# conservation-laws/ryujin

Hardware: AMD Instinct MI355X
Metric: MDoF-updates/s per Euler forward step; achieved HBM GB/s vs roofline (higher is better)
Workload: dtype f64; 1 GPU; 2D Euler Mach-3 forward-facing step, Q1, SSPRK33 stage sequence (BASELINE.json configs[1]); gridpoints_per_gpu=2498844, gridpoints_total=2498844, dofs_total=9995376, cells_per_unit=995, partition=x-slabs x1, equal gridpoint counts, develop_updates=600

## Files before the change

### include/ryujin_hip.h

```cpp
#ifndef RYUJIN_HIP_H
#define RYUJIN_HIP_H

#include <stddef.h>
#include <stdint.h>

#ifdef __cplusplus
extern "C" {
#endif

#define RYUJIN_OK 0
#define RYUJIN_WARN 1
#define RYUJIN_RESTART 2
#define RYUJIN_ERR_TAU (-1)
#define RYUJIN_ERR_ARG (-2)
#define RYUJIN_ERR_HIP (-3)
#define RYUJIN_ERR_COMM (-4)
#define RYUJIN_ERR_UNSUPPORTED (-5)

enum {
  RYUJIN_EQ_EULER = 0,
  RYUJIN_EQ_SHALLOW_WATER = 1,
  RYUJIN_EQ_EULER_AEOS = 2,
  RYUJIN_EQ_SCALAR_CONSERVATION = 3
};

enum { RYUJIN_FLUX_BURGERS = 0, RYUJIN_FLUX_KPP = 1, RYUJIN_FLUX_POLYNOMIAL = 2, RYUJIN_FLUX_FUNCTION = 3 };

enum {
  RYUJIN_EOS_POLYTROPIC_GAS = 0,
  RYUJIN_EOS_NOBLE_ABEL_STIFFENED_GAS = 1,
  RYUJIN_EOS_VAN_DER_WAALS = 2,
  RYUJIN_EOS_JONES_WILKINS_LEE = 3,
  RYUJIN_EOS_FUNCTION = 4
};

enum {
  RYUJIN_BC_DO_NOTHING = 0,
  RYUJIN_BC_PERIODIC = 1,
  RYUJIN_BC_SLIP = 2,
  RYUJIN_BC_NO_SLIP = 3,
  RYUJIN_BC_DIRICHLET = 4,
  RYUJIN_BC_DYNAMIC = 5,
  RYUJIN_BC_DIRICHLET_MOMENTUM = 6
};

enum { RYUJIN_IDV_WARN = 0, RYUJIN_IDV_RAISE_EXCEPTION = 1 };

typedef struct ryujin_hip_params {
  int equation;
  int dim;

  double gamma;
  double reference_density;
  double vacuum_state_relaxation_small;
  double vacuum_state_relaxation_large;

  double gravity;
  double manning_friction_coefficient;
  double reference_water_depth;
  double dry_state_relaxation_factor;
  double dry_state_relaxation_small;
  double dry_state_relaxation_large;

  double cfl;
  int id_violation_strategy;

  double indicator_evc_factor;

  int limiter_iterations;
  double limiter_newton_tolerance;
  int limiter_newton_max_iterations;
  double limiter_relaxation_factor;
  int limiter_limit_on_kinetic_energy;
  int limiter_limit_on_square_velocity;

  int riemann_newton_max_iterations;
  double riemann_newton_tolerance;

  int eos;
  int compute_strict_bounds;
  double eos_covolume_b;
  double eos_q;
  double eos_pinf;
  double eos_vdw_a;
  double eos_gas_constant_R;
  double jwl_A, jwl_B, jwl_R1, jwl_R2, jwl_omega, jwl_rho_0, jwl_q_0, jwl_cv;

  int sc_flux;
  double sc_flux_polynomial[3][4];
  double sc_derivative_approximation_delta;
  int sc_use_greedy_wavespeed;
  int sc_use_averaged_entropy;
  int sc_random_entropies;

  int system_scope_events;
  int debug_join_exchanges;
  int debug_bc_fold_max_slices;
  int debug_no_small_mesh_split;
  int debug_pij_storage;
  int debug_expensive_bounds_check;
  int debug_tile_map;
  int debug_band_stride;
  int debug_xcd_chunk;
  int debug_stencil_classes;
} ryujin_hip_params;

typedef struct ryujin_hip_offline {
  uint32_t n_export, n_internal, n_owned, n_relevant;
  uint32_t simd_length;
  const uint64_t *row_starts;
  const uint32_t *columns;
  const double *cij;
  const double *mij;
  const double *mi;
  const double *mi_inv;
  double measure_of_omega;

  uint32_t n_bdry;
  const uint32_t *b_i;
  const double *b_normal;
  const uint8_t *b_id;

  uint32_t n_pairs;
  const uint32_t *p_i, *p_col, *p_j;

  const double *initial_precomputed;

  int n_nbr;
  const int *nbr_rank;
  const uint32_t *send_off;
  const uint32_t *send_idx;
  const uint32_t *recv_off;
  const uint32_t *row_send_off;
  const uint32_t *row_send_row;
  const uint32_t *row_send_col;

  int discontinuous_ansatz;
  const double *incidence;
  const double *mass_matrix_inverse;
} ryujin_hip_offline;

typedef struct ryujin_hip_ctx ryujin_hip_ctx;

#define RYUJIN_HIP_UNIQUE_ID_BYTES 128
typedef struct ryujin_hip_comm ryujin_hip_comm;
int ryujin_hip_comm_unique_id(char id[RYUJIN_HIP_UNIQUE_ID_BYTES]);
int ryujin_hip_comm_init(ryujin_hip_comm **comm, const char id[RYUJIN_HIP_UNIQUE_ID_BYTES],
                         int rank, int n_ranks, int device);
int ryujin_hip_device_count(int *n_devices);
int ryujin_hip_comm_init_local(ryujin_hip_comm **comms, int n_ranks, int device);
int ryujin_hip_comm_init_loopback(ryujin_hip_comm **comm, int rank, int n_ranks, int device);
void ryujin_hip_comm_destroy(ryujin_hip_comm *comm);
int ryujin_hip_comm_info(const ryujin_hip_comm *comm, int *rank, int *n_ranks, int *rccl_rank,
                         int *rccl_count, int *rccl_device);

void ryujin_hip_default_params(ryujin_hip_params *params, int equation, int dim);

int ryujin_hip_create(ryujin_hip_ctx **ctx, const ryujin_hip_offline *offline,
                      const ryujin_hip_params *params, ryujin_hip_comm *comm, int device);
int ryujin_hip_exchange_info(ryujin_hip_ctx *ctx, int *n_nbr, int *nbr_rank, int max_nbr,
                             unsigned long long *n_exchanges, unsigned long long *n_allreduces);
void ryujin_hip_destroy(ryujin_hip_ctx *ctx);

int ryujin_hip_state_alloc(ryujin_hip_ctx *ctx, int *handle);
int ryujin_hip_state_free(ryujin_hip_ctx *ctx, int handle);
int ryujin_hip_state_upload(ryujin_hip_ctx *ctx, int handle, const double *U_aos);
int ryujin_hip_state_download(ryujin_hip_ctx *ctx, int handle, double *U_aos);
int ryujin_hip_state_download_precomputed(ryujin_hip_ctx *ctx, int handle, double *prec_aos);

int ryujin_hip_host_register(ryujin_hip_ctx *ctx, const void *ptr, size_t bytes);
int ryujin_hip_host_unregister(ryujin_hip_ctx *ctx, const void *ptr);
int ryujin_hip_state_download_owned(ryujin_hip_ctx *ctx, int handle, double *U_aos);
int ryujin_hip_state_download_prepared(ryujin_hip_ctx *ctx, int handle, double *U_aos);

int ryujin_hip_prepare_state_vector(ryujin_hip_ctx *ctx, int handle, double t,
                                    const double *dirichlet_aos);

int ryujin_hip_step(ryujin_hip_ctx *ctx, int h_old, int stages, const int *h_stage,
                    const double *stage_weights, int h_new, double tau_in,
                    double tau_max_in, double *tau_out);

int ryujin_hip_sadd(ryujin_hip_ctx *ctx, int h_dst, double s, double b, int h_src);

enum {
  RYUJIN_SCHEME_SSPRK_22 = 0,
  RYUJIN_SCHEME_SSPRK_33 = 1,
  RYUJIN_SCHEME_ERK_11 = 2,
  RYUJIN_SCHEME_ERK_22 = 3,
  RYUJIN_SCHEME_ERK_33 = 4,
  RYUJIN_SCHEME_ERK_43 = 5,
  RYUJIN_SCHEME_ERK_54 = 6
};
enum { RYUJIN_CFL_RECOVERY_NONE = 0, RYUJIN_CFL_RECOVERY_BANG_BANG = 1 };
int ryujin_hip_time_step(ryujin_hip_ctx *ctx, int scheme, int h_state, const int h_tmp[3],
                         const double *dirichlet_aos, double tau_max, int cfl_recovery, double cfl_min,
                         double cfl_max, double *tau_out);
int ryujin_hip_time_step_n(ryujin_hip_ctx *ctx, int scheme, int h_state, int n_tmp, const int *h_tmp,
                           const double *dirichlet_aos, double tau_max, int cfl_recovery,
                           double cfl_min, double cfl_max, double *tau_out);

typedef void (*ryujin_hip_dirichlet_fn)(void *user, double time, double *dirichlet_aos);
int ryujin_hip_time_step_fn(ryujin_hip_ctx *ctx, int scheme, int h_state, int n_tmp, const int *h_tmp, double t,
                            ryujin_hip_dirichlet_fn dirichlet_fn, void *user, double tau_max, int cfl_recovery,
                            double cfl_min, double cfl_max, double *tau_out);

int ryujin_hip_state_integrals(ryujin_hip_ctx *ctx, int handle, double *out );

int ryujin_hip_set_cfl(ryujin_hip_ctx *ctx, double cfl);
int ryujin_hip_get_cfl(ryujin_hip_ctx *ctx, double *cfl);
int ryujin_hip_set_id_violation_strategy(ryujin_hip_ctx *ctx, int strategy);
int ryujin_hip_get_alpha(ryujin_hip_ctx *ctx, double *alpha );
int ryujin_hip_get_counters(ryujin_hip_ctx *ctx, unsigned *n_restarts, unsigned *n_warnings);
int ryujin_hip_limiter_statistics(ryujin_hip_ctx *ctx, double *limited_slice_fraction, int *pij_stored,
                                  double *stored_slice_fraction);
int ryujin_hip_layout_info(ryujin_hip_ctx *ctx, unsigned long long *n_tiles, unsigned long long *n_regular_tiles);
int ryujin_hip_chain_info(ryujin_hip_ctx *ctx, unsigned long long *n_chained_tiles,
                          unsigned long long *n_chained_entries);
int ryujin_hip_stencil_class_info(ryujin_hip_ctx *ctx, unsigned long long *n_uniform_slices,
                                  unsigned long long *n_classes, double *uniform_entry_fraction);
int ryujin_hip_tile_statistics(ryujin_hip_ctx *ctx, double *stored_fraction, double *read_fraction,
                               double *formed_by_step6_fraction);

int ryujin_hip_debug_fetch(ryujin_hip_ctx *ctx, int what, double *out, size_t n_doubles);
#define RYUJIN_DEBUG_PLAN_LENGTH 32
int ryujin_hip_debug_plan(ryujin_hip_ctx *ctx, int *out, int n);
int ryujin_hip_set_timers(ryujin_hip_ctx *ctx, int enable);
int ryujin_hip_get_timers(ryujin_hip_ctx *ctx, double ms[8]);
int ryujin_hip_get_timers_accum(ryujin_hip_ctx *ctx, double ms[8], unsigned *n_updates, int reset);
int ryujin_hip_synchronize(ryujin_hip_ctx *ctx);
int ryujin_hip_event_record(ryujin_hip_ctx *ctx, int which );
int ryujin_hip_event_elapsed_ms(ryujin_hip_ctx *ctx, double *ms);
int ryujin_hip_debug_layout(const ryujin_hip_offline *offline, uint64_t *ptr, uint32_t *col,
                            uint64_t *transposed, const double *data, uint32_t n_comp, double *out);
int ryujin_hip_debug_addresses(ryujin_hip_ctx *ctx, uint64_t out[8]);
int ryujin_hip_debug_pow(int device, const double *x, const double *y, double *out, size_t n);
enum {
  RYUJIN_DEBUG_EULER_RIEMANN = 0,
  RYUJIN_DEBUG_EULER_LIMIT_1D = 1,
  RYUJIN_DEBUG_SW_RIEMANN = 2,
  RYUJIN_DEBUG_EULER_DIJ_2D = 3,
  RYUJIN_DEBUG_EULER_DIJ_3D = 4,
  RYUJIN_DEBUG_EULER_DIJ_RECORDS_2D = 5,
  RYUJIN_DEBUG_EULER_DIJ_RECORDS_3D = 6,
  RYUJIN_DEBUG_SW_DIJ_2D = 7,
  RYUJIN_DEBUG_SW_DIJ_RECORDS_2D = 8,
  RYUJIN_DEBUG_EULER_RIEMANN_RECORDS = 9,
  RYUJIN_DEBUG_SW_RIEMANN_RECORDS = 10,
  RYUJIN_DEBUG_AEOS_RIEMANN = 11,
  RYUJIN_DEBUG_AEOS_LIMIT_1D = 12,
  RYUJIN_DEBUG_AEOS_DIJ_2D = 13,
  RYUJIN_DEBUG_AEOS_DIJ_RECORDS_2D = 14,
  RYUJIN_DEBUG_EULER_LIMIT_CHECKED_1D = 15,
  RYUJIN_DEBUG_EULER_LIMIT_2D = 16
};
int ryujin_hip_debug_function(int device, const ryujin_hip_params *params, int which, const double *in,
                              double *out, size_t n);
int ryujin_hip_debug_rk_outcome(int restart_accum, int tau_invalid_accum, int id_violation_strategy);
const char *ryujin_hip_last_error(void);
const char *ryujin_hip_version(void);

#define RYUJIN_PP_MAX_QUANTITIES 8
enum { RYUJIN_PP_SCHLIEREN = 0, RYUJIN_PP_VORTICITY = 1 };
typedef struct ryujin_hip_postprocess_quantity {
  int kind;
  int is_primitive;
  int component;
} ryujin_hip_postprocess_quantity;
int ryujin_hip_postprocess_configure(ryujin_hip_ctx *ctx, int n_quantities,
                                     const ryujin_hip_postprocess_quantity *quantities, double beta,
                                     int recompute_bounds);
int ryujin_hip_postprocess_compute(ryujin_hip_ctx *ctx, int state_handle);
int ryujin_hip_postprocess_download(ryujin_hip_ctx *ctx, int q, double *out, int raw);
int ryujin_hip_postprocess_bounds(ryujin_hip_ctx *ctx, int q, double *q_max, double *q_min);

enum { RYUJIN_Q_INSTANTANEOUS = 1, RYUJIN_Q_TIME_AVERAGED = 2, RYUJIN_Q_SPACE_AVERAGED = 4 };
#define RYUJIN_Q_MAX_MANIFOLDS 16
#define RYUJIN_Q_NONE_YET 3
int ryujin_hip_quantities_add_manifold(ryujin_hip_ctx *ctx, uint32_t n_points, const uint32_t *index,
                                       const double *weight, int options, int *manifold_out);
int ryujin_hip_quantities_reset(ryujin_hip_ctx *ctx);
int ryujin_hip_quantities_clear_statistics(ryujin_hip_ctx *ctx);
int ryujin_hip_quantities_accumulate(ryujin_hip_ctx *ctx, int state_handle, double t);
int ryujin_hip_quantities_instantaneous(ryujin_hip_ctx *ctx, int manifold, int state_handle, double t, double *out);
int ryujin_hip_quantities_time_averaged(ryujin_hip_ctx *ctx, int manifold, double *out, double *t_begin,
                                        double *t_end);
int ryujin_hip_quantities_time_series(ryujin_hip_ctx *ctx, int manifold, double *rows, size_t capacity_rows,
                                      size_t *n_rows, int clear);

enum {
  RYUJIN_IV_UNIFORM = 0,
  RYUJIN_IV_RADIAL_CONTRAST = 1,
  RYUJIN_IV_ISENTROPIC_VORTEX = 2,
  RYUJIN_IV_LEBLANC = 3,
  RYUJIN_IV_RAREFACTION = 4,
  RYUJIN_IV_CIRCULAR_DAM_BREAK = 5,
  RYUJIN_IV_PARABOLOID = 6,
  RYUJIN_IV_RITTER_DAM_BREAK = 7,
  RYUJIN_IV_SMOOTH_VORTEX = 8,
  RYUJIN_IV_SLOPING_FRICTION = 9
};
typedef struct ryujin_hip_initial_values {
  int state;
  double params[16];
  double direction[3];
  double position[3];
  double perturbation;
// ... 58 lines not shown
```

### ryujin_amd/capi.py

```python
from __future__ import annotations

import ctypes as C
import os

import numpy as np

from . import _build

c_double_p = C.POINTER(C.c_double)
c_u32_p = C.POINTER(C.c_uint32)
c_u64_p = C.POINTER(C.c_uint64)
c_u8_p = C.POINTER(C.c_uint8)
c_int_p = C.POINTER(C.c_int)

RYUJIN_OK, RYUJIN_WARN, RYUJIN_RESTART = 0, 1, 2
RYUJIN_ERR_TAU, RYUJIN_ERR_ARG, RYUJIN_ERR_HIP, RYUJIN_ERR_COMM, RYUJIN_ERR_UNSUPPORTED = -1, -2, -3, -4, -5
EQ_EULER, EQ_SHALLOW_WATER, EQ_EULER_AEOS, EQ_SCALAR_CONSERVATION = 0, 1, 2, 3
FLUX_BURGERS, FLUX_KPP, FLUX_POLYNOMIAL, FLUX_FUNCTION = 0, 1, 2, 3
EOS_POLYTROPIC_GAS, EOS_NOBLE_ABEL_STIFFENED_GAS, EOS_VAN_DER_WAALS, EOS_JONES_WILKINS_LEE = 0, 1, 2, 3
EOS_FUNCTION = 4
EOS_PRESSURE, EOS_SPECIFIC_INTERNAL_ENERGY, EOS_TEMPERATURE, EOS_SPEED_OF_SOUND = 0, 1, 2, 3
BC_DO_NOTHING, BC_PERIODIC, BC_SLIP, BC_NO_SLIP, BC_DIRICHLET, BC_DYNAMIC, BC_DIRICHLET_MOMENTUM = range(7)
IDV_WARN, IDV_RAISE_EXCEPTION = 0, 1
CUT_NONE, CUT_BOX, CUT_CYLINDER = 0, 1, 2
SCHEME_SSPRK_22, SCHEME_SSPRK_33, SCHEME_ERK_11, SCHEME_ERK_22, SCHEME_ERK_33, SCHEME_ERK_43, SCHEME_ERK_54 = range(7)
CFL_RECOVERY_NONE, CFL_RECOVERY_BANG_BANG = 0, 1
UNIQUE_ID_BYTES = 128
DEBUG_EULER_RIEMANN, DEBUG_EULER_LIMIT_1D, DEBUG_SW_RIEMANN, DEBUG_EULER_DIJ_2D, DEBUG_EULER_DIJ_3D = range(5)
DEBUG_EULER_DIJ_RECORDS_2D, DEBUG_EULER_DIJ_RECORDS_3D = 5, 6
DEBUG_SW_DIJ_2D, DEBUG_SW_DIJ_RECORDS_2D = 7, 8
DEBUG_EULER_RIEMANN_RECORDS, DEBUG_SW_RIEMANN_RECORDS = 9, 10
DEBUG_AEOS_RIEMANN, DEBUG_AEOS_LIMIT_1D = 11, 12
DEBUG_AEOS_DIJ_2D, DEBUG_AEOS_DIJ_RECORDS_2D = 13, 14
DEBUG_EULER_LIMIT_CHECKED_1D, DEBUG_EULER_LIMIT_2D = 15, 16


DIRICHLET_FN = C.CFUNCTYPE(None, C.c_void_p, C.c_double, c_double_p)


class Params(C.Structure):
    _fields_ = [
        ("equation", C.c_int), ("dim", C.c_int),
        ("gamma", C.c_double), ("reference_density", C.c_double),
        ("vacuum_state_relaxation_small", C.c_double), ("vacuum_state_relaxation_large", C.c_double),
        ("gravity", C.c_double), ("manning_friction_coefficient", C.c_double),
        ("reference_water_depth", C.c_double), ("dry_state_relaxation_factor", C.c_double),
        ("dry_state_relaxation_small", C.c_double), ("dry_state_relaxation_large", C.c_double),
        ("cfl", C.c_double), ("id_violation_strategy", C.c_int),
        ("indicator_evc_factor", C.c_double),
        ("limiter_iterations", C.c_int), ("limiter_newton_tolerance", C.c_double),
        ("limiter_newton_max_iterations", C.c_int), ("limiter_relaxation_factor", C.c_double),
        ("limiter_limit_on_kinetic_energy", C.c_int), ("limiter_limit_on_square_velocity", C.c_int),
        ("riemann_newton_max_iterations", C.c_int), ("riemann_newton_tolerance", C.c_double),
        ("eos", C.c_int), ("compute_strict_bounds", C.c_int),
        ("eos_covolume_b", C.c_double), ("eos_q", C.c_double), ("eos_pinf", C.c_double),
        ("eos_vdw_a", C.c_double), ("eos_gas_constant_R", C.c_double),
        ("jwl_A", C.c_double), ("jwl_B", C.c_double), ("jwl_R1", C.c_double), ("jwl_R2", C.c_double),
        ("jwl_omega", C.c_double), ("jwl_rho_0", C.c_double), ("jwl_q_0", C.c_double),
        ("jwl_cv", C.c_double),
        ("sc_flux", C.c_int), ("sc_flux_polynomial", (C.c_double * 4) * 3),
        ("sc_derivative_approximation_delta", C.c_double), ("sc_use_greedy_wavespeed", C.c_int),
        ("sc_use_averaged_entropy", C.c_int), ("sc_random_entropies", C.c_int),
        ("system_scope_events", C.c_int), ("debug_join_exchanges", C.c_int),
        ("debug_bc_fold_max_slices", C.c_int), ("debug_no_small_mesh_split", C.c_int),
        ("debug_pij_storage", C.c_int), ("debug_expensive_bounds_check", C.c_int),
        ("debug_tile_map", C.c_int), ("debug_band_stride", C.c_int),
        ("debug_xcd_chunk", C.c_int), ("debug_stencil_classes", C.c_int),
    ]


class Offline(C.Structure):
    _fields_ = [
        ("n_export", C.c_uint32), ("n_internal", C.c_uint32), ("n_owned", C.c_uint32),
        ("n_relevant", C.c_uint32), ("simd_length", C.c_uint32),
        ("row_starts", c_u64_p), ("columns", c_u32_p), ("cij", c_double_p), ("mij", c_double_p),
        ("mi", c_double_p), ("mi_inv", c_double_p), ("measure_of_omega", C.c_double),
        ("n_bdry", C.c_uint32), ("b_i", c_u32_p), ("b_normal", c_double_p), ("b_id", c_u8_p),
        ("n_pairs", C.c_uint32), ("p_i", c_u32_p), ("p_col", c_u32_p), ("p_j", c_u32_p),
        ("initial_precomputed", c_double_p),
        ("n_nbr", C.c_int), ("nbr_rank", c_int_p), ("send_off", c_u32_p), ("send_idx", c_u32_p),
        ("recv_off", c_u32_p), ("row_send_off", c_u32_p), ("row_send_row", c_u32_p),
        ("row_send_col", c_u32_p),
        ("discontinuous_ansatz", C.c_int), ("incidence", c_double_p), ("mass_matrix_inverse", c_double_p),
    ]


class SynthSpec(C.Structure):
    _fields_ = [
        ("dim", C.c_int), ("n_cells", C.c_uint32 * 3), ("lower", C.c_double * 3),
        ("upper", C.c_double * 3), ("bc", C.c_int * 6), ("cut_kind", C.c_int),
        ("cut_lo", C.c_double * 3), ("cut_hi", C.c_double * 3), ("cyl_center", C.c_double * 2),
        ("cyl_radius", C.c_double), ("cut_bc", C.c_int), ("n_ranks", C.c_int), ("rank", C.c_int),
    ]


PP_SCHLIEREN, PP_VORTICITY = 0, 1
PP_MAX_QUANTITIES = 8
Q_INSTANTANEOUS, Q_TIME_AVERAGED, Q_SPACE_AVERAGED = 1, 2, 4
Q_MAX_MANIFOLDS = 16
Q_NONE_YET = 3
EN_MAX_DOFS_PER_CELL, EN_MAX_POINTS, EN_MAX_COMPONENTS = 27, 64, 5
OUT_MAX_QUANTITIES, OUT_MAX_MANIFOLDS = 32, 8
OUT_FLOAT32, OUT_FLOAT64 = 0, 1


class PostprocessQuantity(C.Structure):
    _fields_ = [("kind", C.c_int), ("is_primitive", C.c_int), ("component", C.c_int)]


(IV_UNIFORM, IV_RADIAL_CONTRAST, IV_ISENTROPIC_VORTEX, IV_LEBLANC, IV_RAREFACTION, IV_CIRCULAR_DAM_BREAK,
 IV_PARABOLOID, IV_RITTER_DAM_BREAK, IV_SMOOTH_VORTEX, IV_SLOPING_FRICTION) = range(10)


class InitialValues(C.Structure):
    _fields_ = [("state", C.c_int), ("params", C.c_double * 16), ("direction", C.c_double * 3),
                ("position", C.c_double * 3), ("perturbation", C.c_double)]


IV_STATES = {
    "uniform": (IV_UNIFORM, False, (("primitive state", 0, (1.4, 3.0, 1.0)),)),
    "radial contrast": (IV_RADIAL_CONTRAST, False, (("primitive state inner", 0, (1.0, 0.0, 100.0)),
                                                    ("primitive state outer", 3, (1.0, 0.0, 0.1)),
                                                    ("radius", 6, 0.5))),
    "isentropic vortex": (IV_ISENTROPIC_VORTEX, False, (("mach number", 0, 2.0), ("beta", 1, 5.0),
                                                        ("gamma", 2, 1.4))),
    "leblanc": (IV_LEBLANC, False, ()),
    "rarefaction": (IV_RAREFACTION, False, (("gamma", 0, 1.4),)),
    "circular dam break": (IV_CIRCULAR_DAM_BREAK, True, (("still water depth", 0, 0.5), ("radius", 1, 2.5),
                                                         ("dam amplitude", 2, 2.5))),
    "paraboloid": (IV_PARABOLOID, True, (("free surface radius", 0, 1.0), ("water height", 1, 0.1),
                                         ("paraboloid length", 2, 10000.0), ("speed", 3, 2.0))),
    "ritter dam break": (IV_RITTER_DAM_BREAK, True, (("time initial", 0, 0.1), ("left water depth", 1, 0.005))),
    "smooth vortex": (IV_SMOOTH_VORTEX, True, (("reference depth", 0, 1.0), ("mach number", 1, 2.0),
                                               ("beta", 2, 0.1))),
    "sloping friction": (IV_SLOPING_FRICTION, True, (("ramp slope", 0, 1.0), ("initial discharge", 1, 0.1))),
}


def initial_values_struct(name: str, dim: int, direction=None, position=None, perturbation: float = 0.0,
                          **params) -> InitialValues:
    if name not in IV_STATES:
        raise ValueError(f"Could not find an initial state description with name \"{name}\"")
    state, _, spec = IV_STATES[name]
    iv = InitialValues()
    iv.state = state
    given = {k.replace("_", " "): v for k, v in params.items()}
    for pname, slot, default in spec:
        value = given.pop(pname, default)
        values = tuple(value) if isinstance(default, tuple) else (value,)
        if len(values) != (len(default) if isinstance(default, tuple) else 1):
# ... 121 lines not shown

def resolve_component(equation: int, dim: int, name: str) -> tuple[int, int]:
    for is_primitive, names in enumerate(component_names(equation, dim)):
        if name in names:
            return is_primitive, names.index(name)
    raise ValueError(f"Invalid component name »{name}«")


def as_ptr(a: np.ndarray, typ):
    return a.ctypes.data_as(typ)


def np_from_ptr(ptr, n: int, dtype) -> np.ndarray:
    if n == 0 or not ptr:
        return np.zeros(0, dtype=dtype)
    return np.ctypeslib.as_array(ptr, shape=(n,)).astype(dtype, copy=True)



_synth = None


def load_synth():
    global _synth
    if _synth is None:
        path = os.environ.get("RYUJIN_SYNTH_LIB", _build.SYNTH_SO)
        if not os.path.exists(path):
            _build.build_synth()
        lib = C.CDLL(path)
        lib.ryujin_synth_build.restype = C.c_void_p
        lib.ryujin_synth_build.argtypes = [C.POINTER(SynthSpec)]
        lib.ryujin_synth_free.argtypes = [C.c_void_p]
        lib.ryujin_synth_last_error.restype = C.c_char_p
        lib.ryujin_synth_offline.restype = C.POINTER(Offline)
        lib.ryujin_synth_offline.argtypes = [C.c_void_p]
        lib.ryujin_synth_nnz.restype = C.c_uint64
        lib.ryujin_synth_nnz.argtypes = [C.c_void_p]
        lib.ryujin_synth_n_global.restype = C.c_uint64
        lib.ryujin_synth_n_global.argtypes = [C.c_void_p]
        lib.ryujin_synth_positions.restype = c_double_p
        lib.ryujin_synth_positions.argtypes = [C.c_void_p]
        lib.ryujin_synth_global_ids.restype = c_u64_p
        lib.ryujin_synth_global_ids.argtypes = [C.c_void_p]
        lib.ryujin_synth_bdry_positions.restype = c_double_p
        lib.ryujin_synth_bdry_positions.argtypes = [C.c_void_p]
        lib.ryujin_synth_bdry_mass.restype = c_double_p
        lib.ryujin_synth_bdry_mass.argtypes = [C.c_void_p]
        lib.ryujin_synth_n_cells.restype = C.c_uint64
        lib.ryujin_synth_n_cells.argtypes = [C.c_void_p]
        lib.ryujin_synth_cells.restype = c_u32_p
        lib.ryujin_synth_cells.argtypes = [C.c_void_p]
        lib.ryujin_synth_ghost_row_send_entries.restype = C.c_size_t
        lib.ryujin_synth_ghost_row_send_entries.argtypes = [c_u64_p, c_u32_p, c_u32_p, C.c_size_t, C.c_uint32,
                                                            C.c_uint32, c_u32_p, c_u32_p]
        lib.ryujin_offline_write.restype = C.c_int
        lib.ryujin_offline_write.argtypes = [C.c_char_p, C.POINTER(Offline), C.c_int, C.c_int, c_double_p,
                                             c_double_p]
        lib.ryujin_offline_read.restype = C.c_void_p
        lib.ryujin_offline_read.argtypes = [C.c_char_p]
        lib.ryujin_offline_file_free.argtypes = [C.c_void_p]
        lib.ryujin_offline_io_last_error.restype = C.c_char_p
        lib.ryujin_offline_file_view.restype = C.POINTER(Offline)
        lib.ryujin_offline_file_view.argtypes = [C.c_void_p]
        lib.ryujin_offline_file_dim.argtypes = [C.c_void_p]
        lib.ryujin_offline_file_n_initial_precomputed.argtypes = [C.c_void_p]
        lib.ryujin_offline_file_nnz.restype = C.c_uint64
        lib.ryujin_offline_file_nnz.argtypes = [C.c_void_p]
        lib.ryujin_offline_file_positions.restype = c_double_p
        lib.ryujin_offline_file_positions.argtypes = [C.c_void_p]
        lib.ryujin_offline_file_b_positions.restype = c_double_p
        lib.ryujin_offline_file_b_positions.argtypes = [C.c_void_p]
        _synth = lib
    return _synth



HIP_SYMBOLS = [
    "ryujin_hip_comm_unique_id", "ryujin_hip_comm_init", "ryujin_hip_comm_init_local",
    "ryujin_hip_comm_init_loopback",
    "ryujin_hip_comm_destroy", "ryujin_hip_comm_info", "ryujin_hip_exchange_info", "ryujin_hip_device_count",
    "ryujin_hip_time_step_fn", "ryujin_hip_debug_addresses",
    "ryujin_hip_host_register", "ryujin_hip_host_unregister", "ryujin_hip_state_download_owned",
    "ryujin_hip_state_download_prepared", "ryujin_hip_layout_info", "ryujin_hip_chain_info", "ryujin_hip_stencil_class_info", "ryujin_hip_tile_statistics",
    "ryujin_hip_default_params", "ryujin_hip_create", "ryujin_hip_destroy",
    "ryujin_hip_state_alloc", "ryujin_hip_state_free", "ryujin_hip_state_upload",
    "ryujin_hip_state_download", "ryujin_hip_state_download_precomputed", "ryujin_hip_state_integrals",
    "ryujin_hip_prepare_state_vector", "ryujin_hip_step", "ryujin_hip_sadd", "ryujin_hip_time_step", "ryujin_hip_time_step_n",
    "ryujin_hip_get_timers_accum",
    "ryujin_hip_set_cfl", "ryujin_hip_get_cfl", "ryujin_hip_set_id_violation_strategy",
    "ryujin_hip_get_alpha", "ryujin_hip_get_counters", "ryujin_hip_limiter_statistics", "ryujin_hip_debug_fetch", "ryujin_hip_debug_plan",
    "ryujin_hip_set_timers", "ryujin_hip_get_timers", "ryujin_hip_synchronize",
    "ryujin_hip_event_record", "ryujin_hip_event_elapsed_ms", "ryujin_hip_last_error",
    "ryujin_hip_version", "ryujin_hip_debug_layout", "ryujin_hip_debug_pow", "ryujin_hip_debug_function", "ryujin_hip_debug_rk_outcome",
    "ryujin_hip_postprocess_configure", "ryujin_hip_postprocess_compute", "ryujin_hip_postprocess_download",
    "ryujin_hip_postprocess_bounds",
    "ryujin_hip_quantities_add_manifold", "ryujin_hip_quantities_reset", "ryujin_hip_quantities_clear_statistics",
    "ryujin_hip_quantities_accumulate", "ryujin_hip_quantities_instantaneous", "ryujin_hip_quantities_time_averaged",
    "ryujin_hip_quantities_time_series",
    "ryujin_hip_initial_values_configure", "ryujin_hip_initial_values_evaluate",
    "ryujin_hip_initial_values_interpolate", "ryujin_hip_prepare_state_vector_iv", "ryujin_hip_time_step_iv",
    "ryujin_hip_initial_values_configure_function", "ryujin_hip_expression_evaluate",
    "ryujin_hip_error_norms_configure", "ryujin_hip_error_norms_compute",
    "ryujin_hip_flux_configure_function", "ryujin_hip_flux_function_evaluate", "ryujin_hip_flux_info",
    "ryujin_hip_eos_configure_function", "ryujin_hip_eos_function_evaluate",
    "ryujin_hip_eos_function_evaluate_device", "ryujin_hip_eos_info",
    "ryujin_hip_output_configure", "ryujin_hip_output_info", "ryujin_hip_output_selection",
    "ryujin_hip_output_levelset_values", "ryujin_hip_output_extract",
]


def _declare_module_api(lib, prefix: str):
    p = lambda n: getattr(lib, prefix + n)
    vp = C.c_void_p
    p("default_params").argtypes = [C.POINTER(Params), C.c_int, C.c_int]
    p("default_params").restype = None
    p("create").argtypes = [C.POINTER(vp), C.POINTER(Offline), C.POINTER(Params), vp, C.c_int]
    p("destroy").argtypes = [vp]
    p("destroy").restype = None
    p("state_alloc").argtypes = [vp, c_int_p]
    p("state_free").argtypes = [vp, C.c_int]
    p("state_upload").argtypes = [vp, C.c_int, c_double_p]
    p("state_download").argtypes = [vp, C.c_int, c_double_p]
    p("state_download_precomputed").argtypes = [vp, C.c_int, c_double_p]
    if hasattr(lib, prefix + "state_integrals"):
        p("state_integrals").argtypes = [vp, C.c_int, c_double_p]
    p("prepare_state_vector").argtypes = [vp, C.c_int, C.c_double, c_double_p]
    p("step").argtypes = [vp, C.c_int, C.c_int, c_int_p, c_double_p, C.c_int, C.c_double,
                          C.c_double, c_double_p]
    p("sadd").argtypes = [vp, C.c_int, C.c_double, C.c_double, C.c_int]
    p("set_cfl").argtypes = [vp, C.c_double]
    p("get_cfl").argtypes = [vp, c_double_p]
    p("set_id_violation_strategy").argtypes = [vp, C.c_int]
    p("get_alpha").argtypes = [vp, c_double_p]
    p("get_counters").argtypes = [vp, C.POINTER(C.c_uint), C.POINTER(C.c_uint)]
    p("debug_fetch").argtypes = [vp, C.c_int, c_double_p, C.c_size_t]
    p("last_error").restype = C.c_char_p


_hip = None


def load_hip():
    global _hip
    if _hip is None:
        path = os.environ.get("RYUJIN_HIP_LIB", _build.HIP_SO)
        if not os.path.exists(path):
            raise RuntimeError(
                f"{path} is missing: build it with `python -m ryujin_amd._build` "
                "(hipcc --offload-arch=gfx950). There is no CPU fallback for the product path.")
        lib = C.CDLL(path, mode=C.RTLD_GLOBAL)
        _declare_module_api(lib, "ryujin_hip_")
        vp = C.c_void_p
        lib.ryujin_hip_comm_unique_id.argtypes = [C.c_char_p]
        lib.ryujin_hip_comm_init.argtypes = [C.POINTER(vp), C.c_char_p, C.c_int, C.c_int, C.c_int]
        lib.ryujin_hip_comm_init_local.argtypes = [C.POINTER(vp), C.c_int, C.c_int]
        lib.ryujin_hip_comm_init_loopback.argtypes = [C.POINTER(vp), C.c_int, C.c_int, C.c_int]
        lib.ryujin_hip_comm_destroy.argtypes = [vp]
        lib.ryujin_hip_comm_destroy.restype = None
        lib.ryujin_hip_comm_info.argtypes = [vp, c_int_p, c_int_p, c_int_p, c_int_p, c_int_p]
        lib.ryujin_hip_exchange_info.argtypes = [vp, c_int_p, c_int_p, C.c_int, C.POINTER(C.c_ulonglong),
                                                 C.POINTER(C.c_ulonglong)]
        lib.ryujin_hip_set_timers.argtypes = [vp, C.c_int]
        lib.ryujin_hip_get_timers.argtypes = [vp, c_double_p]
        lib.ryujin_hip_get_timers_accum.argtypes = [vp, c_double_p, C.POINTER(C.c_uint), C.c_int]
        lib.ryujin_hip_time_step.argtypes = [vp, C.c_int, C.c_int, c_int_p, c_double_p, C.c_double, C.c_int,
                                             C.c_double, C.c_double, c_double_p]
        lib.ryujin_hip_time_step_n.argtypes = [vp, C.c_int, C.c_int, C.c_int, c_int_p, c_double_p, C.c_double,
                                               C.c_int, C.c_double, C.c_double, c_double_p]
        lib.ryujin_hip_time_step_fn.argtypes = [vp, C.c_int, C.c_int, C.c_int, c_int_p, C.c_double, DIRICHLET_FN,
                                                C.c_void_p, C.c_double, C.c_int, C.c_double, C.c_double, c_double_p]
        lib.ryujin_hip_device_count.argtypes = [c_int_p]
        lib.ryujin_hip_layout_info.argtypes = [vp, C.POINTER(C.c_ulonglong), C.POINTER(C.c_ulonglong)]
        lib.ryujin_hip_chain_info.argtypes = [vp, C.POINTER(C.c_ulonglong), C.POINTER(C.c_ulonglong)]
        if hasattr(lib, "ryujin_hip_stencil_class_info"):
            lib.ryujin_hip_stencil_class_info.argtypes = [vp, C.POINTER(C.c_ulonglong), C.POINTER(C.c_ulonglong),
                                                          C.POINTER(C.c_double)]
        lib.ryujin_hip_tile_statistics.argtypes = [vp, C.POINTER(C.c_double), C.POINTER(C.c_double), C.POINTER(C.c_double)]
        lib.ryujin_hip_host_register.argtypes = [vp, C.c_void_p, C.c_size_t]
        lib.ryujin_hip_host_unregister.argtypes = [vp, C.c_void_p]
        lib.ryujin_hip_state_download_owned.argtypes = [vp, C.c_int, c_double_p]
        lib.ryujin_hip_state_download_prepared.argtypes = [vp, C.c_int, c_double_p]
        lib.ryujin_hip_debug_addresses.argtypes = [vp, c_u64_p]
        lib.ryujin_hip_debug_plan.argtypes = [vp, c_int_p, C.c_int]
        lib.ryujin_hip_synchronize.argtypes = [vp]
        lib.ryujin_hip_event_record.argtypes = [vp, C.c_int]
        lib.ryujin_hip_event_elapsed_ms.argtypes = [vp, c_double_p]
        lib.ryujin_hip_version.restype = C.c_char_p
        lib.ryujin_hip_debug_layout.argtypes = [C.POINTER(Offline), c_u64_p, c_u32_p, c_u64_p,
                                                c_double_p, C.c_uint32, c_double_p]
        lib.ryujin_hip_debug_pow.argtypes = [C.c_int, c_double_p, c_double_p, c_double_p, C.c_size_t]
        lib.ryujin_hip_debug_rk_outcome.argtypes = [C.c_int, C.c_int, C.c_int]
        lib.ryujin_hip_debug_function.argtypes = [C.c_int, C.POINTER(Params), C.c_int, c_double_p, c_double_p,
                                                  C.c_size_t]
        lib.ryujin_hip_postprocess_configure.argtypes = [vp, C.c_int, C.POINTER(PostprocessQuantity), C.c_double,
                                                         C.c_int]
        lib.ryujin_hip_postprocess_compute.argtypes = [vp, C.c_int]
        lib.ryujin_hip_postprocess_download.argtypes = [vp, C.c_int, c_double_p, C.c_int]
        lib.ryujin_hip_postprocess_bounds.argtypes = [vp, C.c_int, c_double_p, c_double_p]
        lib.ryujin_hip_quantities_add_manifold.argtypes = [vp, C.c_uint32, c_u32_p, c_double_p, C.c_int, c_int_p]
        lib.ryujin_hip_quantities_reset.argtypes = [vp]
        lib.ryujin_hip_quantities_clear_statistics.argtypes = [vp]
        lib.ryujin_hip_quantities_accumulate.argtypes = [vp, C.c_int, C.c_double]
        lib.ryujin_hip_quantities_instantaneous.argtypes = [vp, C.c_int, C.c_int, C.c_double, c_double_p]
        lib.ryujin_hip_quantities_time_averaged.argtypes = [vp, C.c_int, c_double_p, c_double_p, c_double_p]
        lib.ryujin_hip_quantities_time_series.argtypes = [vp, C.c_int, c_double_p, C.c_size_t,
                                                          C.POINTER(C.c_size_t), C.c_int]
        lib.ryujin_hip_initial_values_configure.argtypes = [vp, C.POINTER(InitialValues), c_double_p, c_double_p]
        lib.ryujin_hip_initial_values_evaluate.argtypes = [vp, c_double_p, C.c_size_t, C.c_double, c_double_p]
        lib.ryujin_hip_initial_values_interpolate.argtypes = [vp, C.c_int, C.c_double]
        lib.ryujin_hip_prepare_state_vector_iv.argtypes = [vp, C.c_int, C.c_double]
        lib.ryujin_hip_time_step_iv.argtypes = [vp, C.c_int, C.c_int, C.c_int, c_int_p, C.c_double, C.c_double,
                                                C.c_int, C.c_double, C.c_double, c_double_p]
        lib.ryujin_hip_initial_values_configure_function.argtypes = [vp, C.c_int, C.POINTER(C.c_char_p), c_double_p,
                                                                     c_double_p, c_double_p, c_double_p]
        lib.ryujin_hip_expression_evaluate.argtypes = [C.c_char_p, C.c_int, c_double_p, C.c_size_t, C.c_double,
                                                       c_double_p]
        lib.ryujin_hip_error_norms_configure.argtypes = [vp, C.c_uint32, C.c_int, c_u32_p, C.c_int, c_double_p,
                                                         c_double_p, c_double_p, C.c_int]
        lib.ryujin_hip_error_norms_compute.argtypes = [vp, C.c_int, C.c_int, C.c_int, c_int_p, C.c_int, c_double_p,
                                                       c_double_p]
        lib.ryujin_hip_flux_configure_function.argtypes = [vp, C.c_char_p, C.c_double]
        lib.ryujin_hip_flux_function_evaluate.argtypes = [C.c_char_p, C.c_int, C.c_double, c_double_p, C.c_size_t,
                                                          c_double_p, c_double_p]
        lib.ryujin_hip_flux_info.argtypes = [vp, c_int_p, c_int_p, c_int_p]
        lib.ryujin_hip_eos_configure_function.argtypes = [vp, C.c_char_p, C.c_char_p, C.c_char_p, C.c_char_p,
                                                          C.c_double, C.c_double, C.c_double]
        lib.ryujin_hip_eos_function_evaluate.argtypes = [C.c_int, C.c_char_p, c_double_p, c_double_p, C.c_size_t,
                                                         c_double_p]
        lib.ryujin_hip_eos_function_evaluate_device.argtypes = [vp, C.c_int, c_double_p, c_double_p, C.c_size_t,
                                                                c_double_p]
        lib.ryujin_hip_eos_info.argtypes = [vp, c_int_p, c_int_p, c_int_p]
        lib.ryujin_hip_output_configure.argtypes = [vp, C.c_int, C.POINTER(C.c_char_p), c_double_p, C.c_uint32, C.c_int,
                                                    c_u32_p, C.c_int, C.POINTER(C.c_char_p)]
        lib.ryujin_hip_output_info.argtypes = [vp, c_u32_p, c_u32_p]
        lib.ryujin_hip_output_selection.argtypes = [vp, c_u32_p, c_u32_p, c_u32_p]
        lib.ryujin_hip_output_levelset_values.argtypes = [vp, C.c_int, c_double_p]
        lib.ryujin_hip_output_extract.argtypes = [vp, C.c_int, C.c_int, C.c_int, C.c_void_p]
        _hip = lib
    return _hip
```

### ryujin_amd/csrc/kernels_euler.hpp

```cpp

#pragma once

#include <hip/hip_runtime.h>

#include <cfloat>
#include <cstdint>

#include "euler_device.hpp"

namespace ryujin_hip
{
  struct DeviceScalars;

  struct StencilClassEntry {
    double c[2];
    double m;
    int32_t delta;
    uint32_t pad;
  };
  static_assert(sizeof(StencilClassEntry) == 32, "four 64-bit words");

  struct StepBegin {
    DeviceScalars *scalars;
    double tau_max_in, tau_in;
// ... 311 lines not shown
    const v4i v = *(const_ptr)(uintptr_t)(M.class_table + e);
    c[0] = uniform_double(v.x, v.y);
    if constexpr (DIM == 2)
      c[1] = uniform_double(v.z, v.w);
  }

  RYUJIN_DEV int32_t class_delta(const DeviceMesh &M, const uint32_t e)
  {
    typedef const int32_t __attribute__((address_space(4))) *const_ptr;
    return __builtin_amdgcn_readfirstlane(*(const_ptr)(uintptr_t)(&M.class_table[e].delta));
  }

  struct TileChain {
    uint32_t kind;
    uint64_t loads;
  };
  template <int DIM>
  constexpr bool chain_masks_pay()
  {
    return DIM == 3;
  }
  template <bool MASKS>
  RYUJIN_DEV TileChain tile_chain(const DeviceMesh &M, const uint64_t colbase)
  {
    TileChain t{kChainNone, ~0ull};
    if (M.tiles != nullptr) {
      typedef const uint32_t __attribute__((address_space(4))) *const_ptr;
      typedef const uint64_t __attribute__((address_space(4))) *const_ptr64;
      const uint32_t code = __builtin_amdgcn_readfirstlane(*(const_ptr)(uintptr_t)&M.tiles[colbase].chain);
      if constexpr (MASKS) {
        t.kind = code & kChainKindMask;
        if (t.kind != kChainNone) {
          const uint64_t m = *(const_ptr64)(uintptr_t)(M.chain_loads + colbase);
          t.loads = ((uint64_t)__builtin_amdgcn_readfirstlane((uint32_t)(m >> 32)) << 32) |
                    (uint64_t)__builtin_amdgcn_readfirstlane((uint32_t)m);
        }
      } else {
        t.kind = (code & kChainEndLaneOnly) != 0u ? (code & kChainKindMask) : kChainNone;
      }
    }
    return t;
  }

  RYUJIN_DEV double lane_next(const double x)
  {
    const int lo = __double2loint(x), hi = __double2hiint(x);
    return __hiloint2double(__builtin_amdgcn_update_dpp(hi, hi, 0x130 , 0xf, 0xf, false),
                            __builtin_amdgcn_update_dpp(lo, lo, 0x130, 0xf, 0xf, false));
  }
  RYUJIN_DEV double lane_prev(const double x)
  {
    const int lo = __double2loint(x), hi = __double2hiint(x);
    return __hiloint2double(__builtin_amdgcn_update_dpp(hi, hi, 0x138 , 0xf, 0xf, false),
                            __builtin_amdgcn_update_dpp(lo, lo, 0x138, 0xf, 0xf, false));
  }
  template <bool MASKS>
  RYUJIN_DEV bool chain_lane_loads(const TileChain &t, const uint32_t lane)
  {
    if constexpr (MASKS)
      return ((t.loads >> lane) & 1ull) != 0ull;
    else
      return lane == (t.kind == kChainOwnPrev ? 0u : 63u);
  }

  RYUJIN_DEV uint32_t tile_transposed(const DeviceMesh &M, const TileDesc &t, const uint64_t colbase,
                                      const uint32_t lane)
  {
    if (t.delta != kTileIrregular)
      return (lane < 64u - ((uint32_t)t.delta & 63u) ? t.ta : t.tb) + lane;
    uint32_t pos = M.idx_t[colbase * 64 + lane];
    asm volatile("" : "+v"(pos));
    return pos;
  }

  template <bool USE = true>
  RYUJIN_DEV uint32_t tile_transposed(const DeviceMesh &M, const uint64_t colbase, const uint32_t lane)
  {
    return tile_transposed(M, tile_desc<USE>(M, colbase), colbase, lane);
  }

  RYUJIN_DEV void batch_fence() { __builtin_amdgcn_sched_barrier(0); }

  template <bool USE, int N>
  RYUJIN_DEV void transposed_positions(const DeviceMesh &M, const RowCtx &r, const int c0, uint32_t (&tpos)[N])
  {
    if constexpr (USE) {
      if (M.tiles != nullptr) {
        int4 raw[N];
#pragma unroll
        for (int k = 0; k < N; ++k) {
          raw[k] = int4{kTileIrregular, 0, 0, 0};
          if ((uint32_t)(c0 + k) < r.width)
            raw[k] = load_tile_desc(M.tiles + ((uint64_t)r.base + c0 + k));
        }
        batch_fence();
        bool any_irregular = false;
#pragma unroll
        for (int k = 0; k < N; ++k) {
          tpos[k] = 0;
          if ((uint32_t)(c0 + k) < r.width) {
            const int32_t delta = __builtin_amdgcn_readfirstlane(raw[k].x);
            const uint32_t ta = (uint32_t)__builtin_amdgcn_readfirstlane(raw[k].y);
            const uint32_t tb = (uint32_t)__builtin_amdgcn_readfirstlane(raw[k].z);
            tpos[k] = (r.lane < 64u - ((uint32_t)delta & 63u) ? ta : tb) + r.lane;
            any_irregular = any_irregular || delta == kTileIrregular;
          }
        }
        if (any_irregular) {
#pragma unroll
          for (int k = 0; k < N; ++k)
            if ((uint32_t)(c0 + k) < r.width && __builtin_amdgcn_readfirstlane(raw[k].x) == kTileIrregular)
              tpos[k] = M.idx_t[((uint64_t)r.base + c0 + k) * 64 + r.lane];
        }
#pragma unroll
        for (int k = 0; k < N; ++k)
          asm volatile("" : "+v"(tpos[k]));
        return;
      }
    }
#pragma unroll
    for (int k = 0; k < N; ++k) {
      tpos[k] = 0;
      if ((uint32_t)(c0 + k) < r.width)
        tpos[k] = M.idx_t[((uint64_t)r.base + c0 + k) * 64 + r.lane];
    }
#pragma unroll
    for (int k = 0; k < N; ++k)
      asm volatile("" : "+v"(tpos[k]));
  }

  RYUJIN_DEV void arrived(double &x) { asm volatile("" : "+v"(x)); }
  RYUJIN_DEV void arrived(uint32_t &x) { asm volatile("" : "+v"(x)); }
  template <int N>
  RYUJIN_DEV void arrived(double (&x)[N])
  {
#pragma unroll
    for (int q = 0; q < N; ++q)
      arrived(x[q]);
  }

  RYUJIN_DEV uint32_t mapped_block(const DeviceMesh &M)
  {
    uint32_t block = blockIdx.x;
    if (M.xcd_chunk > 0u) {
      const uint32_t span = 8u * M.xcd_chunk;
      if (block < gridDim.x - gridDim.x % span) {
        const uint32_t rem = block % span;
        block = block - rem + (rem & 7u) * M.xcd_chunk + (rem >> 3);
      }
    }
    return block;
  }

  RYUJIN_DEV RowCtx row_context(const DeviceMesh &M)
  {
    RowCtx r;
    r.lane = threadIdx.x & 63;
    const uint32_t block = mapped_block(M);
    uint32_t id = block * kWavesPerBlock + (uint32_t)__builtin_amdgcn_readfirstlane(threadIdx.x >> 6);
    if (M.band_stride > 1u) {
      const uint32_t band = kWavesPerBlock * M.band_stride;
      const uint32_t n = M.slice_end - M.slice_begin;
      if (id < n - n % band) {
        const uint32_t rem = id % band;
        id = id - rem + rem / kWavesPerBlock + (rem % kWavesPerBlock) * M.band_stride;
      }
    }
    r.slice = __builtin_amdgcn_readfirstlane(M.slice_begin + id);
    r.valid = r.slice < M.slice_end;
    if (!r.valid) {
      r.row = r.len = r.base = r.width = 0;
      return r;
    }
    r.row = r.slice * 64 + r.lane;
    r.len = M.row_len[r.row];
    r.base = __builtin_amdgcn_readfirstlane(M.slice_off[r.slice]);
    r.width = __builtin_amdgcn_readfirstlane(M.slice_off[r.slice + 1]) - r.base;
    return r;
  }


  struct BcFold {
    const unsigned long long *slice_mask;
    const uint32_t *slice_first;
    const uint32_t *grp_start;
    const double *b_normal;
    const uint8_t *b_id;
    const double *dirichlet;
  };

  template <typename E>
  RYUJIN_DEV void apply_bc_group(const typename E::Params &P, const BcFold &B, const uint32_t g, const uint32_t i,
                                 double *U)
  {
    constexpr int K = E::K;
    constexpr int DIM = E::DIMENSION;
    const uint32_t e0 = B.grp_start[g], e1 = B.grp_start[g + 1];
    double U_i[K];
    load_state<K>(U, i, U_i);
    bool touched = false;
    for (uint32_t e = e0; e < e1; ++e) {
      const int id = B.b_id[e];
      if (id == RYUJIN_BC_DO_NOTHING)
        continue;
      double normal[DIM], U_D[K], result[K];
#pragma unroll
// ... 934 lines not shown
```

### ryujin_amd/csrc/kernels_limiter.hpp

```cpp

#pragma once

#include "kernels_euler.hpp"


namespace ryujin_hip
{
  RYUJIN_DEV double lmin(const double a, const double b)
  {
    return (a == a && b == b) ? fmin(a, b) : a + b;
  }

  RYUJIN_DEV void flag_restart(DeviceScalars *scalars, const bool all_ok, const uint32_t lane)
  {
    if (__any(!all_ok)) {
      if (lane == 0)
        atomicOr(&scalars->restart_needed, 1);
    }
  }

  template <typename E>
  struct TailScratch {
    static constexpr int kRowDoubles = (E::NB + E::K) * 64;
    double rows[kRowDoubles];
// ... 636 lines not shown
          if (!__any(active && !(old_l_ij == 1.))) {
            if (active)
              st_stream(lij_next + (pos), 0.);
            continue;
          }
          double p_ij[K];
          load_entry<K>(pij, colbase, r.lane, p_ij);
          if (!active)
            continue;
          double new_p_ij[K];
#pragma unroll
          for (int q = 0; q < K; ++q)
            new_p_ij[q] = (1. - old_l_ij) * p_ij[q];
          bool success, undecided;
          const double new_l_ij =
              E::limit_fast(P, bnd, U_i_new, new_p_ij, success, undecided);
          if (undecided)
            undecided_mask |= 1ull << (c - c_blk + 1);
          else
            st_stream(lij_next + (pos), (1. - old_l_ij) * new_l_ij);
        }
        limit_undecided_pairs<E>(
            P, r, undecided_mask, bnd, U_i_new, tail_queue + (threadIdx.x >> 6) * 63 * 64,
            tail_rows[threadIdx.x >> 6].rows,
            [&](const uint32_t c, const uint32_t owner, double (&out)[K]) {
              const uint64_t pos = ((uint64_t)r.base + c) * 64 + owner;
              const double old_l_ij = lmin(lij[pos], lij[idx_t[pos]]);
              load_entry<K>(pij, (uint64_t)r.base + c, owner, out);
#pragma unroll
              for (int q = 0; q < K; ++q)
                out[q] = (1. - old_l_ij) * out[q];
            },
            [&](const uint32_t c, const uint32_t owner, const double new_l_ij) {
              const uint64_t pos = ((uint64_t)r.base + c) * 64 + owner;
              const double old_l_ij = lmin(lij[pos], lij[idx_t[pos]]);
              st_stream(lij_next + (pos), (1. - old_l_ij) * new_l_ij);
            },
            c_blk - 1);
        undecided_mask = 0;
        if constexpr (!WIDE)
          break;
      }
    }
  }

  template <int K>
  RYUJIN_DEV void repair_missing_tiles(const uint32_t *__restrict__ cols, const double *__restrict__ mij,
                                       const double *__restrict__ mi_inv, const double *__restrict__ old_U,
                                       const double *__restrict__ r_in, const double *__restrict__ alpha,
                                       const double *__restrict__ dij, const double tau, const uint32_t i,
                                       const uint32_t len, const uint32_t base, const uint32_t width,
                                       const uint32_t lane, const bool row_active, const uint32_t missing,
                                       double *__restrict__ pij)
  {
    RowData<K> row;
    load_state<K>(old_U, i, row.U_i);
    load_state<K>(r_in, i, row.F_i);
    row.alpha_i = alpha[i];
    row.m_i_inv = mi_inv[i];
    row.factor = tau * row.m_i_inv * (double)(len - 1);
#pragma unroll 1
    for (uint32_t c = 1; c < width; ++c) {
      if (!((missing >> c) & 1u))
        continue;
      const uint64_t pos = ((uint64_t)base + c) * 64 + lane;
      const uint32_t j = cols[pos];
      PairData<K> pd;
      pd.d_ij = dij[pos];
      pd.m_ij = ld_stream(mij + pos);
      load_state<K>(old_U, j, pd.U_j);
      load_state<K>(r_in, j, pd.F_j);
      pd.alpha_j = alpha[j];
      pd.m_j_inv = mi_inv[j];
      double P_t[K];
      pij_stage0<K>(row, pd, P_t);
      if (row_active && c < len)
        store_entry<K>(pij, (uint64_t)base + c, lane, P_t);
    }
  }

  struct SliceFlags {
    uint8_t *unlimited, *first_stored, *todo;
    uint32_t *needed_tiles;
  };

#ifndef RYUJIN_GATHER_GROUP_3D
#define RYUJIN_GATHER_GROUP_3D 6
#endif
  template <int MAXW>
  RYUJIN_DEV uint32_t tiles_predicted(const SliceFlags &W, const uint32_t slice)
  {
    static_assert(MAXW <= 10, "P_ij per tile up to two dimensions");
    const uint32_t word = W.needed_tiles[slice];
    uint32_t m = word & 0x3ffu;
    m |= (word >> 10) & 0x3ffu;
    m |= (word >> 20) & 0x3ffu;
    return m;
  }
  template <int MAXW>
  RYUJIN_DEV void tiles_remember(const SliceFlags &W, const uint32_t slice, const uint32_t needed)
  {
    static_assert(MAXW <= 10, "P_ij per tile up to two dimensions");
    W.needed_tiles[slice] = ((W.needed_tiles[slice] << 10) | (needed & 0x3ffu)) & 0x3fffffffu;
  }

  template <int K>
  RYUJIN_DEV void backfill_pij(const DeviceMesh &M, const Stage0Src &S0, const RowCtx &r,
                               double *__restrict__ pij, const uint32_t c_end)
  {
    if (r.len <= 1)
      return;
    RowData<K> row;
    load_row_data<K>(M, S0, r.row, r.len, row);
    for (uint32_t c = 1; c < c_end && c < r.len; ++c) {
      double P_ij[K];
      pij_on_the_fly<K>(M, S0, row, (uint64_t)r.base + c, r.lane, P_ij);
      store_entry<K>(pij, (uint64_t)r.base + c, r.lane, P_ij);
    }
  }

  template <typename E, int MAXW, int CHUNK>
  RYUJIN_DEV void last_cached_slice(const typename E::Params &P, const DeviceMesh &M, const RowCtx &r,
                                    double *__restrict__ new_U, const double *__restrict__ pij,
                                    const double *__restrict__ lij, const FusedSadd &F, const FusedPrecompute &FP,
                                    const uint8_t *__restrict__ slice_unlimited = nullptr)
  {
    constexpr int K = E::K;
    const bool row_active = r.len > 1;
    const uint32_t i = row_active ? r.row : (r.row < M.n_owned ? r.row : M.n_owned - 1);
    const uint32_t *__restrict__ idx_t = M.idx_t;

    double U_i_new[K];
    load_state<K>(new_U, i, U_i_new);
    double V[K];
    if (F.src)
      load_state<K>(F.src, i, V);
    const double lambda = 1. / (double)(r.len - 1);

    double l[MAXW];
    uint32_t needed = 0;
    const bool known_unlimited = slice_unlimited != nullptr && slice_unlimited[r.slice] != 0;
#pragma unroll
    for (int c = 1; c < MAXW; ++c)
      l[c] = 0.;
    if (!known_unlimited) {
      constexpr int CH = MAXW - 1 < 9 ? MAXW - 1 : RYUJIN_GATHER_GROUP_3D;
#pragma unroll
      for (int c0 = 1; c0 < MAXW; c0 += CH) {
        uint32_t tpos[CH];
        transposed_positions<tile_map_pays<E::DIMENSION>(), CH>(M, r, c0, tpos);
        batch_fence();
        double l_a[CH], l_b[CH];
#pragma unroll
        for (int k = 0; k < CH; ++k) {
          const int c = c0 + k;
          l_a[k] = l_b[k] = 0.;
          if (c < MAXW && (uint32_t)c < r.width) {
            l_a[k] = lij[(uint32_t)(((uint64_t)r.base + c) * 64 + r.lane)];
            l_b[k] = lij[tpos[k]];
          }
        }
        batch_fence();
#pragma unroll
        for (int k = 0; k < CH; ++k) {
          asm volatile("" : "+v"(l_a[k]));
          asm volatile("" : "+v"(l_b[k]));
        }
#pragma unroll
        for (int k = 0; k < CH; ++k) {
          const int c = c0 + k;
          if (c < MAXW && (uint32_t)c < r.width)
            l[c] = (row_active && (uint32_t)c < r.len) ? lmin(l_a[k], l_b[k]) : 0.;
        }
      }
#pragma unroll
      for (int c = 1; c < MAXW; ++c)
        if (__any(l[c] != 0.))
          needed |= 1u << c;
    }

#pragma unroll
    for (int c0 = 1; c0 < MAXW; c0 += CHUNK) {
      double p[CHUNK][K];
#pragma unroll
      for (int cc = 0; cc < CHUNK; ++cc) {
        const int c = c0 + cc;
        if (c < MAXW && ((needed >> c) & 1u))
          load_entry<K>(pij, (uint64_t)r.base + c, r.lane, p[cc]);
      }
#pragma unroll
      for (int cc = 0; cc < CHUNK; ++cc) {
        const int c = c0 + cc;
        if (c < MAXW && ((needed >> c) & 1u)) {
          if (row_active && (uint32_t)c < r.len) {
#pragma unroll
            for (int q = 0; q < K; ++q)
              U_i_new[q] += l[c] * lambda * p[cc][q];
          }
        }
      }
    }

    if (F.src) {
#pragma unroll
      for (int q = 0; q < K; ++q)
        U_i_new[q] = F.s * U_i_new[q] + F.b * V[q];
    }
    if (row_active || (F.src != nullptr && r.row < M.n_owned))
      store_state<K>(new_U, i, U_i_new);
    if (FP.prec != nullptr && row_active)
      fused_precompute<E>(P, FP, i, U_i_new);
  }

  RYUJIN_DEV RowCtx row_context_of_slice(const DeviceMesh &M, const uint32_t slice)
  {
    RowCtx r;
    r.lane = threadIdx.x & 63;
    r.slice = slice;
    r.valid = true;
    r.row = slice * 64 + r.lane;
    r.len = M.row_len[r.row];
    r.base = M.slice_off[slice];
    r.width = M.slice_off[slice + 1] - r.base;
    return r;
  }

  template <typename E, int MAXW, int CHUNK>
  __global__ void __launch_bounds__(kBlock, (MAXW > 9 ? RYUJIN_OCC_LAST_3D : 1))
  k_high_order_last_cached(const typename E::Params P, const DeviceMesh M, double *__restrict__ new_U,
                           const double *__restrict__ pij, const double *__restrict__ lij, const FusedSadd F,
                           const FusedPrecompute FP, const uint8_t *__restrict__ slice_unlimited = nullptr)
  {
    const RowCtx r = row_context(M);
    if (!r.valid)
      return;
    last_cached_slice<E, MAXW, CHUNK>(P, M, r, new_U, pij, lij, F, FP, slice_unlimited);
  }

  constexpr int kHoPlain = 0, kHoLight = 1, kHoHeavy = 2;
  template <int DIM, int MODE>
  constexpr bool forms_missing_tiles()
  {
    return DIM <= 2 && MODE == kHoPlain;
  }

  template <typename E, int MAXW, int CP, bool SPLIT, int MODE>
  RYUJIN_DEV void next_cached_slice(const typename E::Params &P, const DeviceMesh &M, const RowCtx &r,
                                    const uint32_t group, double *__restrict__ new_U,
                                    const double *__restrict__ bounds, double *__restrict__ pij,
                                    const double *__restrict__ lij, double *__restrict__ lij_next,
                                    const double *__restrict__ V_unlimited, const Stage0Src &S0, const SliceFlags &W,
                                    const uint32_t todo = 1)
  {
    constexpr int K = E::K;
    constexpr int NB = E::NB;
    static_assert(!SPLIT || CP == MAXW, "the split variant caches the whole row");
    static_assert(!SPLIT || MODE == kHoPlain, "small meshes keep the stored P_ij");
    const bool row_active = r.len > 1;
    const uint32_t i = row_active ? r.row : (r.row < M.n_owned ? r.row : M.n_owned - 1);
    const uint32_t *__restrict__ idx_t = M.idx_t;

    double l[MAXW];
    if constexpr (MODE == kHoLight) {
      bool limited = false;
      constexpr int CH = MAXW - 1 < 9 ? MAXW - 1 : RYUJIN_GATHER_GROUP_3D;
#pragma unroll
      for (int c0 = 1; c0 < MAXW; c0 += CH) {
        uint32_t tpos[CH];
        transposed_positions<tile_map_pays<E::DIMENSION>(), CH>(M, r, c0, tpos);
        batch_fence();
        double l_a[CH], l_b[CH];
#pragma unroll
        for (int k = 0; k < CH; ++k) {
          const int c = c0 + k;
          l_a[k] = l_b[k] = 1.;
          if (c < MAXW && (uint32_t)c < r.width) {
            l_a[k] = lij[(uint32_t)(((uint64_t)r.base + c) * 64 + r.lane)];
            l_b[k] = lij[tpos[k]];
          }
        }
        batch_fence();
#pragma unroll
        for (int k = 0; k < CH; ++k) {
          asm volatile("" : "+v"(l_a[k]));
          asm volatile("" : "+v"(l_b[k]));
        }
#pragma unroll
        for (int k = 0; k < CH; ++k) {
          const int c = c0 + k;
          if (c < MAXW && (uint32_t)c < r.width)
            limited = limited || (row_active && (uint32_t)c < r.len && !(l_a[k] == 1. && l_b[k] == 1.));
        }
      }
      const bool slice_limited = __any(limited);
      if ((r.slice & 15u) == 0 && r.lane == 0) {
        atomicAdd(&S0.scalars->n_sampled_slices, 1u);
        if (slice_limited)
          atomicAdd(&S0.scalars->n_sampled_limited, 1u);
      }
      if (r.lane == 0) {
        W.todo[r.slice] = slice_limited ? 3 : 0;
        if (!slice_limited)
          W.unlimited[r.slice] = 1;
      }
      if (!slice_limited && row_active) {
        double V_i[K];
        load_state<K>(V_unlimited, i, V_i);
        store_state<K>(new_U, i, V_i);
#pragma unroll
        for (int c = 1; c < MAXW; ++c)
          if ((uint32_t)c < r.len)
            st_stream(lij_next + ((r.base + c) * 64 + r.lane), 0.);
      }
      return;
    }

    double U_i_new[K];
    const double lambda = 1. / (double)(r.len - 1);
    const size_t stride = M.bounds_stride;
    double bnd[NB];
#pragma unroll
    for (int b = 0; b < NB; ++b)
      bnd[b] = bounds[(size_t)b * stride + i];

    double p[CP][K];
    uint32_t needed = 0;
    uint32_t own_limited = 0;
    if (V_unlimited != nullptr) {
      constexpr bool kTileMode = forms_missing_tiles<E::DIMENSION, MODE>() && !SPLIT;
      const bool tiles = kTileMode && S0.tile_store != 0 && W.needed_tiles != nullptr;
      uint32_t predicted = 0u;
      if constexpr (kTileMode)
        predicted = tiles ? tiles_predicted<MAXW>(W, r.slice) : 0u;
      bool limited = false;
      auto fetch_l = [&](const uint32_t lane) {
        needed = own_limited = 0u;
        constexpr int CH = MAXW - 1 < 9 ? MAXW - 1 : RYUJIN_GATHER_GROUP_3D;
        RowCtx rr = r;
        rr.lane = lane;
#pragma unroll
        for (int c0 = 1; c0 < MAXW; c0 += CH) {
          uint32_t tpos[CH];
          transposed_positions<tile_map_pays<E::DIMENSION>(), CH>(M, rr, c0, tpos);
          batch_fence();
          double l_a[CH], l_b[CH];
#pragma unroll
          for (int k = 0; k < CH; ++k) {
            const int c = c0 + k;
            l_a[k] = l_b[k] = 1.;
            if (c < MAXW && (uint32_t)c < r.width) {
              l_a[k] = lij[(uint32_t)(((uint64_t)r.base + c) * 64 + lane)];
              l_b[k] = lij[tpos[k]];
            }
          }
          batch_fence();
#pragma unroll
          for (int k = 0; k < CH; ++k) {
            asm volatile("" : "+v"(l_a[k]));
            asm volatile("" : "+v"(l_b[k]));
          }
#pragma unroll
          for (int k = 0; k < CH; ++k) {
            const int c = c0 + k;
            if (c >= MAXW)
              continue;
            l[c] = 1.;
            if ((uint32_t)c < r.width) {
              const bool lane_on = row_active && (uint32_t)c < r.len;
              const bool lim = lane_on && !(l_a[k] == 1. && l_b[k] == 1.);
              l[c] = lane_on ? lmin(l_a[k], l_b[k]) : 1.;
              limited = limited || lim;
              if (__any(lim))
                needed |= 1u << c;
              if (__any(lane_on && !(l_a[k] == 1.)))
                own_limited |= 1u << c;
            }
          }
        }
      };
      fetch_l(r.lane);
      const bool slice_limited = needed != 0u;
      (void)limited;
      const uint32_t missing = (kTileMode && S0.tile_store != 0) ? (needed & ~(own_limited | predicted)) : 0u;
      if (S0.scalars != nullptr && (r.slice & 15u) == 0 && r.lane == 0 && (!SPLIT || group == 0) &&
          !(MODE == kHoHeavy && todo == 3)) {
        atomicAdd(&S0.scalars->n_sampled_slices, 1u);
        if (slice_limited)
          atomicAdd(&S0.scalars->n_sampled_limited, 1u);
      }
      if (W.unlimited != nullptr && r.lane == 0 && (!SPLIT || group == 0))
        W.unlimited[r.slice] = slice_limited ? 0 : 1;
      if constexpr (kTileMode)
        if (tiles && r.lane == 0 && (!SPLIT || group == 0))
          tiles_remember<MAXW>(W, r.slice, needed);
      load_state<K>(V_unlimited, i, U_i_new);
      if (!slice_limited) {
        if (row_active) {
          if (!SPLIT || group == 0)
            store_state<K>(new_U, i, U_i_new);
#pragma unroll
          for (int c = 1; c < MAXW; ++c)
            if ((uint32_t)c < r.len && (!SPLIT || (uint32_t)(c - 1) % kWavesPerBlock == group))
              st_stream(lij_next + ((r.base + c) * 64 + r.lane), 0.);
        }
        return;
      }
      if (kTileMode && tiles && (r.slice & 15u) == 0 && r.lane == 0 && (!SPLIT || group == 0)) {
        atomicAdd(&S0.scalars->n_sampled_tiles_needed, (unsigned int)__popc(needed));
        atomicAdd(&S0.scalars->n_sampled_tiles_formed, (unsigned int)__popc(missing));
      }
      if constexpr (kTileMode) {
        if (missing != 0u)
          repair_missing_tiles<K>(M.cols, M.mij, M.mi_inv, S0.old_U, S0.r_in, S0.alpha, S0.dij, S0.scalars->tau, i,
                                  r.len, r.base, r.width, r.lane, row_active, missing, pij);
      }
      if constexpr (E::kLimitedUpdateFromV) {
        const uint32_t row_cols = row_active ? ((r.len >= 32u ? 0xffffffffu : ((1u << r.len) - 1u)) & ~1u) : 0u;
        const bool ref_order = row_active && (needed & row_cols) == row_cols;
        if (__any(ref_order)) {
          double U_low[K];
          load_state<K>(new_U, i, U_low);
#pragma unroll
          for (int q = 0; q < K; ++q)
            U_i_new[q] = ref_order ? U_low[q] : U_i_new[q];
        }
#pragma unroll
        for (int c = 1; c < CP; ++c) {
#pragma unroll
          for (int q = 0; q < K; ++q)
            p[c][q] = 0.;
          if ((needed >> c) & 1u)
            load_entry<K>(pij, (uint64_t)r.base + c, r.lane, p[c]);
        }
#pragma unroll
        for (int c = 1; c < MAXW; ++c) {
          if (!((needed >> c) & 1u))
            continue;
          const double w = (row_active && (uint32_t)c < r.len) ? (ref_order ? l[c] : l[c] - 1.) : 0.;
          if (c < CP) {
#pragma unroll
            for (int q = 0; q < K; ++q)
              U_i_new[q] += w * lambda * p[c < CP ? c : 0][q];
          } else {
            double pt[K];
            load_entry<K>(pij, (uint64_t)r.base + c, r.lane, pt);
#pragma unroll
            for (int q = 0; q < K; ++q)
              U_i_new[q] += w * lambda * pt[q];
          }
        }
      } else {
        load_state<K>(new_U, i, U_i_new);
#pragma unroll
        for (int c = 1; c < CP; ++c) {
#pragma unroll
          for (int q = 0; q < K; ++q)
            p[c][q] = 0.;
          if ((uint32_t)c < r.width)
            load_entry<K>(pij, (uint64_t)r.base + c, r.lane, p[c]);
        }
#pragma unroll
        for (int c = 1; c < MAXW; ++c) {
          if (c < CP) {
            if (row_active && (uint32_t)c < r.len) {
#pragma unroll
              for (int q = 0; q < K; ++q)
                U_i_new[q] += l[c] * lambda * p[c < CP ? c : 0][q];
            }
          } else if ((uint32_t)c < r.width) {
            double pt[K];
            load_entry<K>(pij, (uint64_t)r.base + c, r.lane, pt);
            if (row_active && (uint32_t)c < r.len) {
#pragma unroll
              for (int q = 0; q < K; ++q)
                U_i_new[q] += l[c] * lambda * pt[q];
            }
          }
        }
      }
    } else {
      load_state<K>(new_U, i, U_i_new);
#pragma unroll
      for (int c = 1; c < MAXW; ++c) {
        l[c] = 0.;
        if (c < CP) {
#pragma unroll
          for (int q = 0; q < K; ++q)
            p[c < CP ? c : 0][q] = 0.;
        }
        if ((uint32_t)c < r.width) {
          const uint64_t colbase = (uint64_t)r.base + c;
          const uint32_t pos = (uint32_t)(colbase * 64 + r.lane);
          const double l_a = lij[pos];
          const double l_b = lij[tile_transposed<tile_map_pays<E::DIMENSION>()>(M, (uint64_t)r.base + c, r.lane)];
          l[c] = lmin(l_a, l_b);
          if (c < CP)
            load_entry<K>(pij, colbase, r.lane, p[c < CP ? c : 0]);
          if (__any(row_active && (uint32_t)c < r.len && !(l[c] == 1.)))
            needed |= 1u << c;
        }
      }
#pragma unroll
      for (int c = 1; c < MAXW; ++c) {
        if (c < CP) {
          if (row_active && (uint32_t)c < r.len) {
#pragma unroll
            for (int q = 0; q < K; ++q)
              U_i_new[q] += l[c] * lambda * p[c < CP ? c : 0][q];
          }
        } else if ((uint32_t)c < r.width) {
          double pt[K];
          load_entry<K>(pij, (uint64_t)r.base + c, r.lane, pt);
          if (row_active && (uint32_t)c < r.len) {
#pragma unroll
            for (int q = 0; q < K; ++q)
              U_i_new[q] += l[c] * lambda * pt[q];
          }
        }
      }
    }
    if constexpr (SPLIT) {
      __syncthreads();
      if (row_active && group == 0)
        store_state<K>(new_U, i, U_i_new);
    } else {
      if (row_active)
        store_state<K>(new_U, i, U_i_new);
    }

    unsigned long long undecided_mask = 0;
#pragma unroll
    for (int c = 1; c < MAXW; ++c) {
      if ((uint32_t)c >= r.width)
        continue;
      if (SPLIT && (uint32_t)(c - 1) % kWavesPerBlock != group)
        continue;
      const bool lane_on = row_active && (uint32_t)c < r.len;
      if (!((needed >> c) & 1u)) {
        if (lane_on)
          st_stream(lij_next + ((r.base + c) * 64 + r.lane), 0.);
        continue;
      }
      double pc[K];
      if (c < CP) {
#pragma unroll
        for (int q = 0; q < K; ++q)
          pc[q] = p[c < CP ? c : 0][q];
      } else {
        load_entry<K>(pij, (uint64_t)r.base + c, r.lane, pc);
      }
      if (lane_on) {
        double new_p_ij[K];
#pragma unroll
        for (int q = 0; q < K; ++q)
          new_p_ij[q] = (1. - l[c]) * pc[q];
        bool success, undecided;
        const double new_l_ij =
            E::limit_fast(P, bnd, U_i_new, new_p_ij, success, undecided);
        if (undecided)
          undecided_mask |= 1ull << c;
        else
          st_stream(lij_next + ((r.base + c) * 64 + r.lane), (1. - l[c]) * new_l_ij);
      }
    }
    __shared__ uint16_t tail_queue[kWavesPerBlock * (MAXW - 1) * 64];
    __shared__ TailScratch<E> tail_rows[kWavesPerBlock];
    limit_undecided_pairs<E>(
        P, r, undecided_mask, bnd, U_i_new, tail_queue + (threadIdx.x >> 6) * (MAXW - 1) * 64,
        tail_rows[threadIdx.x >> 6].rows,
        [&](const uint32_t c, const uint32_t owner, double (&out)[K]) {
          const uint64_t pos = ((uint64_t)r.base + c) * 64 + owner;
          const double old_l_ij = lmin(lij[pos], lij[idx_t[pos]]);
          load_entry<K>(pij, (uint64_t)r.base + c, owner, out);
#pragma unroll
          for (int q = 0; q < K; ++q)
            out[q] = (1. - old_l_ij) * out[q];
        },
        [&](const uint32_t c, const uint32_t owner, const double new_l_ij) {
          const uint64_t pos = ((uint64_t)r.base + c) * 64 + owner;
          const double old_l_ij = lmin(lij[pos], lij[idx_t[pos]]);
          st_stream(lij_next + (pos), (1. - old_l_ij) * new_l_ij);
        });
  }

  template <typename E>
  __global__ void __launch_bounds__(kBlock)
  k_pij_repair(const DeviceMesh M, const Stage0Src S0, double *__restrict__ pij, const SliceFlags W)
  {
    const uint32_t slice = M.slice_begin + blockIdx.x * kWavesPerBlock + (threadIdx.x >> 6);
    if (slice >= M.slice_end || W.todo[slice] < 2)
      return;
    const uint32_t fs = W.first_stored[slice];
    const RowCtx r = row_context_of_slice(M, slice);
    backfill_pij<E::K>(M, S0, r, pij, fs == 0 ? 0xffffffffu : fs);
    if (r.lane == 0)
      W.first_stored[slice] = 1;
  }

  template <typename E, int MAXW, int CP = MAXW, bool SPLIT = false, int MODE = kHoPlain>
  __global__ void __launch_bounds__(kBlock, (MAXW > 9 ? (CP < MAXW ? RYUJIN_OCC_HO_3D : 1) : RYUJIN_OCC_HO))
  k_high_order_next_cached(const typename E::Params P, const DeviceMesh M, double *__restrict__ new_U,
                           const double *__restrict__ bounds, double *__restrict__ pij,
                           const double *__restrict__ lij, double *__restrict__ lij_next,
                           const double *__restrict__ V_unlimited = nullptr, const Stage0Src S0 = Stage0Src{},
                           const SliceFlags W = SliceFlags{})
  {
    RowCtx r;
    const uint32_t group = SPLIT ? (threadIdx.x >> 6) : 0u;
    uint32_t todo = 1;
    if constexpr (SPLIT) {
      if (M.slice_begin + blockIdx.x >= M.slice_end)
        return;
      r = row_context_of_slice(M, M.slice_begin + blockIdx.x);
    } else if constexpr (MODE == kHoLight || MODE == kHoHeavy) {
      const uint32_t slice = M.slice_begin + mapped_block(M) * kWavesPerBlock + (threadIdx.x >> 6);
      if (slice >= M.slice_end)
        return;
      if constexpr (MODE == kHoLight) {
        const uint32_t fs = W.first_stored[slice];
        if (fs != 0) {
          if ((threadIdx.x & 63) == 0)
            W.todo[slice] = fs == 1 ? 1 : 2;
          return;
        }
      } else {
        todo = W.todo[slice];
        if (todo == 0)
          return;
      }
      r = row_context_of_slice(M, slice);
    } else {
      r = row_context(M);
      if (!r.valid)
        return;
    }
    next_cached_slice<E, MAXW, CP, SPLIT, MODE>(P, M, r, group, new_U, bounds, pij, lij, lij_next, V_unlimited, S0,
                                                W, todo);
  }
}
```

### ryujin_amd/csrc/ryujin_hip.hip

```cpp

#include <hip/hip_runtime.h>
#include <rccl/rccl.h>

#include <algorithm>
#include <atomic>
#include <cmath>
#include <cstddef>
#include <cstdlib>
#include <cstring>
#include <condition_variable>
#include <limits>
#include <memory>
#include <mutex>
#include <numeric>
#include <string>
#include <type_traits>
#include <vector>

#include "ryujin_hip.h"

#ifndef RYUJIN_XCD_CHUNK_3D
#define RYUJIN_XCD_CHUNK_3D 8
#endif

// ... 371 lines not shown
    DeviceBuffer<uint32_t> d_cell_dofs;
    DeviceBuffer<double> d_jxw;
    DeviceBuffer<double> d_shape, d_weights;
    DeviceBuffer<double> d_work;
  };
  std::unique_ptr<ErrorNorms> error_norms;
  void error_norms_compute(int h_state, int h_analytic, const ErrorNormsDesc &D, double *host_result);
  struct Output {
    OutputDesc desc{};
    bool needs_precomputed = false, needs_postprocessed = false;
    int n_postprocess = 0, pp_kind[kPostprocessMaxQuantities] = {}, pp_select[kPostprocessMaxQuantities] = {};
    int n_manifolds = 0, dofs_per_cell = 0;
    uint32_t n_cells = 0, n_selected_cells = 0, n_selected_nodes = 0;
    DeviceBuffer<double> d_levelsets;
    DeviceBuffer<uint32_t> d_cell_ids, d_node_ids, d_connectivity;
    DeviceBuffer<double> d_columns;
    DeviceBuffer<OutputDesc> d_desc;
    DeviceBuffer<unsigned char> d_out;
  };
  std::unique_ptr<Output> output;
  template <typename E>
  void output_extract(Output &o, int h, bool levelsets, bool float64, void *host_out);
  static constexpr int kMaxRkStages = 5;
  unsigned long long *h_tau_early = nullptr;
  hipEvent_t ev_tau = nullptr;
  bool want_tau_early = false;
  double *h_dirichlet_stage[kMaxRkStages] = {};
  bool iv_configured = false;
  InitialValuesParams iv{};
  DeviceBuffer<double> d_iv_positions, d_iv_b_positions;
  DeviceBuffer<IvFunctionProgram> d_iv_function;
  DeviceBuffer<double> d_iv_points, d_iv_values;
  struct IvStage {
    bool on;
    double t, c;
  };
  void require_initial_values() const
  {
    if (!iv_configured)
      throw HipError(RYUJIN_ERR_ARG, "initial values: not configured (ryujin_hip_initial_values_configure)");
  }
  template <typename E>
  void initial_values_points(const double *d_points, size_t n, double t, int stride, double *d_out);

  struct State {
    DeviceBuffer<double> U, prec;
    DeviceBuffer<double> rrec;
    bool used = false;
    bool precomputed = false;
    bool prepared = false;
  };
  std::vector<std::unique_ptr<State>> states;

  ExchangeTables exch;
  DeviceBuffer<uint32_t> d_send_idx, d_row_send_pos;
  DeviceBuffer<double> d_send_buf;

  DeviceBuffer<double> d_V;
  StepPlan last_plan{};
  Stage0Src last_s0{};
  struct LaunchRecord {
    uint32_t n_slices = 0, grid_y = 0;
    bool shares_slices = false;
  };
  struct LaunchLog {
    static constexpr int kParts = 2;
    int n_step5 = 0, n_step6 = 0;
    LaunchRecord step5[kParts], step6[kParts];
  } last_launches{};
  void record_step5(const DeviceMesh &mm, const uint32_t grid_y)
  {
    if (last_launches.n_step5 < LaunchLog::kParts)
      last_launches.step5[last_launches.n_step5] = LaunchRecord{mm.slice_end - mm.slice_begin, grid_y, false};
    ++last_launches.n_step5;
  }
  void record_step6(const DeviceMesh &mm, const uint32_t grid_y, const bool shares_slices)
  {
    if (last_launches.n_step6 < LaunchLog::kParts)
      last_launches.step6[last_launches.n_step6] = LaunchRecord{mm.slice_end - mm.slice_begin, grid_y, shares_slices};
    ++last_launches.n_step6;
  }
  DeviceBuffer<uint8_t> d_slice_unlimited, d_slice_first_stored, d_slice_todo;
  DeviceBuffer<uint32_t> d_slice_needed;
  double limited_fraction = 1., stored_fraction = 1.;
  unsigned int seen_sampled_slices = 0, seen_sampled_limited = 0, seen_sampled_stored = 0;
  unsigned int seen_sampled_tiles = 0, seen_sampled_tiles_stored = 0;
  unsigned int seen_sampled_tiles_needed = 0, seen_sampled_tiles_formed = 0;
  double tiles_needed_fraction = 1., tiles_formed_fraction = 0.;
  void update_limited_fraction()
  {
    const unsigned int d_tiles = h_scalars->n_sampled_tiles - seen_sampled_tiles;
    const unsigned int d_tiles_stored = h_scalars->n_sampled_tiles_stored - seen_sampled_tiles_stored;
    seen_sampled_tiles = h_scalars->n_sampled_tiles;
    seen_sampled_tiles_stored = h_scalars->n_sampled_tiles_stored;
    const unsigned int d_slices = h_scalars->n_sampled_slices - seen_sampled_slices;
    const unsigned int d_limited = h_scalars->n_sampled_limited - seen_sampled_limited;
    const unsigned int d_stored = h_scalars->n_sampled_stored - seen_sampled_stored;
    seen_sampled_slices = h_scalars->n_sampled_slices;
    seen_sampled_limited = h_scalars->n_sampled_limited;
    seen_sampled_stored = h_scalars->n_sampled_stored;
    if (d_slices != 0) {
      limited_fraction = (double)d_limited / (double)d_slices;
      stored_fraction = last_plan.per_slice() ? (double)d_stored / (double)d_slices : 1.;
    }
    const unsigned int d_needed = h_scalars->n_sampled_tiles_needed - seen_sampled_tiles_needed;
    const unsigned int d_formed = h_scalars->n_sampled_tiles_formed - seen_sampled_tiles_formed;
    seen_sampled_tiles_needed = h_scalars->n_sampled_tiles_needed;
    seen_sampled_tiles_formed = h_scalars->n_sampled_tiles_formed;
    if (last_plan.per_tile() && d_tiles != 0) {
      stored_fraction = (double)d_tiles_stored / (double)d_tiles;
      tiles_needed_fraction = (double)d_needed / (double)d_tiles;
      tiles_formed_fraction = (double)d_formed / (double)d_tiles;
    }
  }
  void ensure_pij()
  {
    if (d_pij.n == 0)
      d_pij.alloc(L.nnz_total * (size_t)K);
  }
  template <typename E>
  void store_pij_for_debug();

  unsigned n_restarts = 0, n_warnings = 0;
  unsigned long long n_exchanges = 0, n_allreduces = 0;

  bool timers_enabled = false;
  bool deferred = false;
  int rk_stage = 0;
  double sweep_ms_accum[8] = {};
  unsigned sweep_updates_accum = 0;
  hipEvent_t ev_rk[5][9] = {};
  hipEvent_t ev[9] = {};
  hipEvent_t ev_user[2] = {};
  double sweep_ms[8] = {};

  ~ryujin_hip_ctx()
  {
    if (stream)
      (void)hipStreamSynchronize(stream);
    if (comm_stream) {
      (void)hipStreamSynchronize(comm_stream);
      (void)hipStreamDestroy(comm_stream);
    }
    if (ev_prev)
      (void)hipEventDestroy(ev_prev);
    if (ev_exp)
      (void)hipEventDestroy(ev_exp);
    if (ev_comm)
      (void)hipEventDestroy(ev_comm);
    for (auto &e : ev)
      if (e)
        (void)hipEventDestroy(e);
    for (auto &set : ev_rk)
      for (auto &e : set)
        if (e)
          (void)hipEventDestroy(e);
    for (auto &e : ev_user)
      if (e)
        (void)hipEventDestroy(e);
    if (h_scalars)
      (void)hipHostFree(h_scalars);
    if (h_bc_pack)
      (void)hipHostFree(h_bc_pack);
    for (const void *ptr : registered_host)
      (void)hipHostUnregister(const_cast<void *>(ptr));
    if (h_tau_early)
// ... 635 lines not shown
                             launch_stream, eparams, mm, bc, d_eos_function.ptr, s.U.ptr, s.prec.ptr, s.rrec.ptr,
                             d_gamma.ptr);
        });
      } else
        with_bool(fold_bc, [&](auto fold) {
          hipLaunchKernelGGL((k_precompute_aeos0<E::DIMENSION, decltype(fold)::value>), grid, block, 0, launch_stream,
                             eparams, mm, bc, s.U.ptr, s.prec.ptr, s.rrec.ptr, d_gamma.ptr);
        });
    });
    exchange_vector(s.U.ptr, KP, true);
    exchange_vector(s.prec.ptr, 4, true);
    if (L.n_relevant > L.n_owned) {
      hipLaunchKernelGGL(k_ghost_records_aeos<E::DIMENSION>, dim3(grid_for(L.n_relevant - L.n_owned)), block, 0,
                         exch.n_nbr ? comm_stream : stream, eparams, L.n_owned, L.n_relevant, s.U.ptr, s.prec.ptr,
                         s.rrec.ptr, d_gamma.ptr);
      if (exch.n_nbr) {
        comm_pending = true;
        exchange_after_exp = true;
      }
    }
    sweep([&](const DeviceMesh &mm, dim3 grid) {
      hipLaunchKernelGGL(k_precompute_aeos1<E::DIMENSION>, grid, block, 0, launch_stream, eparams, mm, s.U.ptr,
                         d_gamma.ptr, s.prec.ptr, s.prec.ptr);
    });
    exchange_vector(s.prec.ptr, 4, true);
  } else if constexpr (std::is_same<typename E::Params, ScalarParams>::value) {
    sweep([&](const DeviceMesh &mm, dim3 grid) {
      if (eparams.flux == RYUJIN_FLUX_FUNCTION) {
        const dim3 slices(mm.slice_end - mm.slice_begin), wave(kFluxFunctionBlock);
        with_bool(fold_bc, [&](auto fold) {
          hipLaunchKernelGGL((k_precompute_sc_function<E::DIMENSION, decltype(fold)::value>), slices, wave, 0,
                             launch_stream, eparams, mm, bc, d_flux_function.ptr, s.U.ptr, s.prec.ptr);
        });
      } else
        with_bool(fold_bc, [&](auto fold) {
          hipLaunchKernelGGL((k_precompute_sc<E::DIMENSION, decltype(fold)::value>), grid, block, 0, launch_stream,
                             eparams, mm, bc, s.U.ptr, s.prec.ptr);
        });
    });
    exchange_vector(s.U.ptr, KP, true);
    exchange_vector(s.prec.ptr, E::NPREC, true);
  } else {
    static_assert(std::is_same<typename E::Params, EulerParams>::value ||
                      std::is_same<typename E::Params, ShallowWaterParams>::value,
                  "Descriptions with node records");
    if (have_records) {
      exchange_vector(s.U.ptr, KP, bdry.n_groups == 0);
    } else {
      sweep([&](const DeviceMesh &mm, dim3 grid) {
        with_bool(fold_bc, [&](auto fold) {
          hipLaunchKernelGGL((k_precompute_records<E, decltype(fold)::value>), grid, block, 0, launch_stream, eparams,
                             mm, bc, s.U.ptr, s.prec.ptr, s.rrec.ptr);
        });
      });
      exchange_vector(s.U.ptr, KP, true);
    }
    if (L.n_relevant > L.n_owned) {
      hipLaunchKernelGGL(k_ghost_precompute_records<E>, dim3(grid_for(L.n_relevant - L.n_owned)), block, 0,
                         exch.n_nbr ? comm_stream : stream, eparams, L.n_owned, L.n_relevant, s.U.ptr, s.prec.ptr,
                         s.rrec.ptr);
      if (exch.n_nbr) {
        comm_pending = true;
        exchange_after_exp = true;
      }
    }
  }
  HIP_CHECK(hipGetLastError());
}

template <typename E>
StepPlanInput ryujin_hip_ctx::plan_input(const int stages) const
{
  StepPlanInput in;
  in.equation = is_euler_v<E> ? PlanEquation::euler
                              : (is_aeos_v<E> ? PlanEquation::euler_aeos
                                              : (is_scalar_v<E> ? PlanEquation::scalar : PlanEquation::shallow_water));
  in.dim = E::DIMENSION;
  in.fusable_precompute = E::kFusablePrecompute;
  in.stages = stages;
  in.limiter_iterations = params.limiter_iterations;
  in.dg = dg;
  in.max_row_len = L.max_row_len;
  in.n_slices = L.n_slices;
  in.debug_pij_storage = params.debug_pij_storage;
  in.checked = params.debug_expensive_bounds_check != 0;
  in.limited_fraction = limited_fraction;
  in.per_slice_max_limited = (double)RYUJIN_PER_SLICE_MAX_LIMITED;
  in.resident_waves_step5 = resident_waves_step5;
  in.resident_waves_step6 = resident_waves_step6;
  in.bc_fold_max_slices = bc_fold_max_slices;
  in.pending_precompute = pending_precompute;
  in.riemann_newton_max_iterations = eparams.riemann_newton_max_iterations;
  in.rarefaction_power = eparams.rarefaction_power;
  in.friction = swparams.manning != 0.;
  return in;
}

template <typename E>
void ryujin_hip_ctx::step2_dij_alpha(const StepPlan &plan, const State &old)
{
  constexpr int DIM = E::DIMENSION;
  const auto &eparams = eq_params<E>();
  const dim3 block(kBlock);
  if constexpr (is_aeos_v<E>) {
    sweep([&](const DeviceMesh &mm, dim3 grid) {
      hipLaunchKernelGGL(k_alpha_aeos<DIM>, grid, block, 0, launch_stream, eparams, mm, old.U.ptr, old.prec.ptr,
                         d_alpha.ptr);
    });
    mark(8);
    exchange_vector(d_alpha.ptr, 1, true);
    sweep([&](const DeviceMesh &mm, dim3 grid) {
      hipLaunchKernelGGL(k_dij_aeos<DIM>, grid, block, 0, launch_stream, eparams, mm, d_lower_mask.ptr,
                         old.rrec.ptr, d_dij.ptr);
    });
  } else if constexpr (is_scalar_v<E>) {
    const bool interpreted = flux_interpreted_pairs();
    last_flux_kind = eparams.flux;
    last_flux_n_instructions = eparams.flux == RYUJIN_FLUX_FUNCTION ? flux_n_instructions : 0;
    last_step2_interpreted = interpreted ? 1 : 0;
    sweep([&](const DeviceMesh &mm, dim3 grid) {
      if (interpreted)
        hipLaunchKernelGGL(k_dij_alpha_sc_function<DIM>, grid, block, 0, launch_stream, eparams, mm,
                           d_flux_function.ptr, old.U.ptr, old.prec.ptr, d_dij.ptr, d_alpha.ptr);
      else
        hipLaunchKernelGGL(k_dij_alpha_sc<DIM>, grid, block, 0, launch_stream, eparams, mm, old.U.ptr,
                           old.prec.ptr, d_dij.ptr, d_alpha.ptr);
    });
    mark(8);
    exchange_vector(d_alpha.ptr, 1, true);
  } else if (plan.step2 == StepPlan::Step2::records) {
    sweep([&](const DeviceMesh &mm, dim3 grid) {
      hipLaunchKernelGGL((k_dij_alpha_records<E, false>), grid, block, 0, launch_stream, eparams, mm,
                         old.U.ptr, old.prec.ptr, old.rrec.ptr, d_dij.ptr, d_alpha.ptr);
    });
    exchange_vector(d_alpha.ptr, 1, true);
  } else if (plan.step2 == StepPlan::Step2::alpha_then_dij) {
    sweep([&](const DeviceMesh &mm, dim3 grid) {
      hipLaunchKernelGGL(k_alpha<E>, grid, block, 0, launch_stream, eparams, mm, old.U.ptr, old.prec.ptr,
                         d_alpha.ptr);
    });
    mark(8);
    exchange_vector(d_alpha.ptr, 1, true);
    sweep([&](const DeviceMesh &mm, dim3 grid) {
      if constexpr (is_euler_v<E>)
        with_bool(!plan.fast_riemann, [&](auto newton) {
          hipLaunchKernelGGL((k_dij_records<E, decltype(newton)::value>), grid, block, 0, launch_stream, eparams, mm,
                             d_lower_mask.ptr, old.rrec.ptr, d_dij.ptr);
        });
    });
  } else {
    sweep([&](const DeviceMesh &mm, dim3 grid) {
      hipLaunchKernelGGL(k_dij_alpha<E>, grid, block, 0, launch_stream, eparams, mm, old.U.ptr,
                         old.prec.ptr, d_dij.ptr, d_alpha.ptr);
    });
    exchange_vector(d_alpha.ptr, 1, true);
  }
}

template <typename E>
void ryujin_hip_ctx::step3_diagonal_tau(const StepPlan &plan, const State &old)
{
  constexpr int DIM = E::DIMENSION;
  const auto &eparams = eq_params<E>();
  const dim3 block(kBlock);
  if (const uint32_t n_pairs = (uint32_t)d_p_pos.n) {
    join_export();
    if constexpr (is_aeos_v<E>)
      hipLaunchKernelGGL(k_dij_boundary_aeos<DIM>, dim3(grid_for(n_pairs)), block, 0, stream, eparams,
                         n_pairs, d_p_i.ptr, d_p_j.ptr, d_p_pos.ptr, d_p_cji.ptr, old.rrec.ptr, d_dij.ptr);
    else if constexpr (is_scalar_v<E>) {
      if (flux_interpreted_pairs())
        hipLaunchKernelGGL(k_dij_boundary_sc_function<DIM>, dim3(grid_for(n_pairs, kFluxFunctionBlock)),
                           dim3(kFluxFunctionBlock), 0, stream, eparams, d_flux_function.ptr, n_pairs, d_p_i.ptr,
                           d_p_j.ptr, d_p_pos.ptr, d_p_cji.ptr, old.U.ptr, old.prec.ptr, d_dij.ptr);
      else
        hipLaunchKernelGGL(k_dij_boundary_sc<DIM>, dim3(grid_for(n_pairs)), block, 0, stream, eparams,
                           n_pairs, d_p_i.ptr, d_p_j.ptr, d_p_pos.ptr, d_p_cji.ptr, old.U.ptr,
                           old.prec.ptr, d_dij.ptr);
    }
    else
      hipLaunchKernelGGL(k_dij_boundary<E>, dim3(grid_for(n_pairs)), block, 0, stream, eparams,
                         n_pairs, d_p_i.ptr, d_p_j.ptr, d_p_pos.ptr, d_p_cji.ptr, old.U.ptr, d_dij.ptr);
  }
  sweep([&](const DeviceMesh &mm, dim3 grid) {
    auto unrolled = [&](auto width) {
      hipLaunchKernelGGL(k_dij_diag_unrolled<decltype(width)::value>, grid, block, 0, launch_stream, mm,
                         d_lower_mask.ptr, params.cfl, d_dij.ptr, d_scalars.ptr);
    };
    if (plan.diag_width == 3)
      unrolled(std::integral_constant<int, 3>{});
    else if (plan.diag_width == 9)
      unrolled(std::integral_constant<int, 9>{});
    else if (plan.diag_width == 27)
      unrolled(std::integral_constant<int, 27>{});
    else
      hipLaunchKernelGGL(k_dij_diag, grid, block, 0, launch_stream, mm, params.cfl, d_dij.ptr,
                         d_scalars.ptr);
  });
  if (!(deferred && rk_stage > 0))
    allreduce_scalar(&d_scalars.ptr->tau_max_bits, 0);
  if (want_tau_early && deferred && rk_stage == 0) {
    join_export();
    HIP_CHECK(hipMemcpyAsync(h_tau_early, &d_scalars.ptr->tau_max_bits, sizeof(unsigned long long),
                             hipMemcpyDeviceToHost, stream));
    HIP_CHECK(hipEventRecord(ev_tau, stream));
  }
}

void ryujin_hip_ctx::ensure_limiter_buffers(const StepPlan &plan)
{
  if (params.limiter_iterations == 2 && d_V.n == 0) {
    d_V.alloc((size_t)L.n_relevant * KP);
    d_slice_unlimited.alloc(L.n_slices);
  }
  ensure_pij();
  if (plan.per_slice() && d_slice_first_stored.n == 0) {
    d_slice_first_stored.alloc(L.n_slices);
    d_slice_todo.alloc(L.n_slices);
  }
  if (plan.tiles_predicted_from_history && d_slice_needed.n == 0) {
    d_slice_needed.alloc(L.n_slices);
    HIP_CHECK(hipMemsetAsync(d_slice_needed.ptr, 0xff, (size_t)L.n_slices * sizeof(uint32_t), launch_stream));
  }
}

template <typename E>
void ryujin_hip_ctx::step4_low_order(const StepPlan &plan, const StepArgs<E::DIMENSION> &a)
{
  constexpr int DIM = E::DIMENSION;
  const auto &eparams = eq_params<E>();
  const dim3 block(kBlock);
  const State &old = a.old, &nw = a.nw;
  sweep([&](const DeviceMesh &mm, dim3 grid) {
    auto launch = [&](auto kernel, auto... bathymetry) {
      hipLaunchKernelGGL(kernel, grid, block, 0, launch_stream, eparams, mm, d_scalars.ptr, a.weight, a.S, old.U.ptr,
                         old.prec.ptr, bathymetry..., d_alpha.ptr, d_dij.ptr, nw.U.ptr, d_r.ptr, d_bounds.ptr,
                         d_pij.ptr);
    };
    if constexpr (is_sw_v<E>) {
      if (plan.step4_single_walk) {
        constexpr int kSwWidth = DIM == 1 ? 3 : 9;
        return with_bool(plan.step4_has_stages, [&](auto has_stages) {
          with_bool(plan.step4_friction, [&](auto friction) {
            launch(k_low_order_sw_single_walk<DIM, decltype(has_stages)::value, kSwWidth, decltype(friction)::value>,
                   d_Z.ptr);
          });
        });
      }
    }
    auto launch4 = [&](auto has_stages, auto stores_p, auto dg_) {
      constexpr bool HS = decltype(has_stages)::value, SP = decltype(stores_p)::value, DG = decltype(dg_)::value;
      if constexpr (is_euler_v<E>)
        launch(k_low_order<DIM, HS, SP, DG>);
      else if constexpr (is_aeos_v<E>)
        launch(k_low_order_aeos<DIM, HS, SP, DG>);
      else if constexpr (is_scalar_v<E>)
        launch(k_low_order_sc<DIM, HS, DG>);
      else
        launch(k_low_order_sw<DIM, HS, DG>, d_Z.ptr);
    };
    if (!plan.step4_stores_p)
      launch4(std::false_type{}, std::false_type{}, std::false_type{});
    else
      with_bool(plan.step4_has_stages, [&](auto has_stages) {
        with_bool(plan.dg, [&](auto dg_) { launch4(has_stages, std::true_type{}, dg_); });
      });
  });
  if (plan.checked)
    sweep([&](const DeviceMesh &mm, dim3 grid) {
      hipLaunchKernelGGL(k_check_admissible<E>, grid, block, 0, launch_stream, eparams, mm, d_scalars.ptr,
                         (const double *)nw.U.ptr);
    });
  exchange_vector(d_r.ptr, KP, true);
  if (plan.dg && plan.step5 != StepPlan::Step5::none) {
    for (int b = 0; b < NB; ++b)
      exchange_vector(d_bounds.ptr + (size_t)b * mesh.bounds_stride, 1, true);
  }
}

template <typename E>
void ryujin_hip_ctx::step5_limiter(const StepPlan &plan, const StepArgs<E::DIMENSION> &a)
{
  using Step5 = StepPlan::Step5;
  constexpr int DIM = E::DIMENSION;
  const auto &eparams = eq_params<E>();
  const dim3 block(kBlock);
  const State &old = a.old, &nw = a.nw;
  if (plan.step5 == Step5::none)
    return;
  if (plan.dg) {
    sweep([&](const DeviceMesh &mm, dim3 grid) {
      if constexpr (is_euler_v<E>)
        hipLaunchKernelGGL(k_bounds_combine_euler, grid, block, 0, launch_stream, mm, d_bounds.ptr,
                           d_bounds_combined.ptr);
      else if constexpr (is_sw_v<E>)
        hipLaunchKernelGGL(k_bounds_combine_sw, grid, block, 0, launch_stream, mm, d_bounds.ptr,
                           d_bounds_combined.ptr);
      else if constexpr (is_aeos_v<E>)
        hipLaunchKernelGGL((k_bounds_combine_minmax<4, 0x2u>), grid, block, 0, launch_stream, mm, d_bounds.ptr,
                           d_bounds_combined.ptr);
      else
        hipLaunchKernelGGL((k_bounds_combine_minmax<2, 0x2u>), grid, block, 0, launch_stream, mm, d_bounds.ptr,
                           d_bounds_combined.ptr);
    });
    std::swap(d_bounds.ptr, d_bounds_combined.ptr);
  }
// ... 10 lines not shown
      constexpr std::integral_constant<int, 1> one{};
      if (plan.step5 == Step5::stage0_per_tile) {
        if constexpr (DIM <= 2)
          stage0(one, std::false_type{}, std::true_type{}, a.tile_flags, 0);
        return;
      }
      if (plan.step5 == Step5::stage0_per_slice)
        return stage0(one, std::true_type{}, std::false_type{}, a.slice_flags, params.debug_pij_storage);
      if (plan.step5 == Step5::stage0_groups)
        return with_groups(plan.step5_groups,
                           [&](auto ny) { stage0(ny, std::false_type{}, std::false_type{}, a.tile_flags, 0); });
    }
    if constexpr (is_euler_v<E>) {
      if (plan.step5 == Step5::recompute) {
        with_groups(plan.recompute_groups(grid.x), [&](auto ny) {
          constexpr int NY = decltype(ny)::value;
          hipLaunchKernelGGL((k_pij_lij_recompute<DIM, NY>), dim3(grid.x, NY), block, 0, launch_stream, eparams,
                             mm, d_scalars.ptr, a.weight, old.U.ptr, d_alpha.ptr, d_dij.ptr, nw.U.ptr, d_r.ptr,
                             d_bounds.ptr, d_pij.ptr, d_lij.ptr);
          record_step5(mm, NY);
        });
        return;
      }
    }
    with_bool(plan.dg, [&](auto dg_) {
      with_bool(plan.wide, [&](auto wide) {
        hipLaunchKernelGGL((k_pij_lij<E, decltype(dg_)::value, decltype(wide)::value>), grid, block,
                           tail_queue_bytes(mm), launch_stream, eparams, mm, d_scalars.ptr, nw.U.ptr, d_r.ptr,
                           d_bounds.ptr, d_pij.ptr, d_lij.ptr, d_V.ptr);
      });
    });
    record_step5(mm, 1);
  });
  if (plan.checked)
    sweep([&](const DeviceMesh &mm, dim3 grid) {
      hipLaunchKernelGGL(k_check_limiter<E>, grid, block, 0, launch_stream, eparams, mm, d_scalars.ptr,
                         (const double *)nw.U.ptr, (const double *)d_bounds.ptr, (const double *)d_pij.ptr,
                         (const double *)nullptr);
    });
  exchange_matrix(d_lij.ptr, true);
}

template <typename E>
void ryujin_hip_ctx::step6_high_order_next(const StepPlan &plan, const StepArgs<E::DIMENSION> &a)
{
  using Step6 = StepPlan::Step6;
  constexpr int DIM = E::DIMENSION;
  constexpr int kWidth = q1_stencil_width(DIM);
  constexpr int kCachedP =
      DIM == 3 ? RYUJIN_HO_CP_3D : (DIM == 2 ? (RYUJIN_HO_CP_2D < kWidth ? RYUJIN_HO_CP_2D : kWidth) : kWidth);
  const auto &eparams = eq_params<E>();
  const dim3 block(kBlock);
  const State &nw = a.nw;
  double *const V = plan.has_V ? d_V.ptr : nullptr;
  uint8_t *const unlimited = plan.has_V ? d_slice_unlimited.ptr : nullptr;
  sweep([&](const DeviceMesh &mm, dim3 grid) {
    if constexpr (is_euler_v<E> || is_aeos_v<E>) {
      if (plan.step6 == Step6::per_slice) {
        auto launch_mode = [&](auto mode) {
          hipLaunchKernelGGL((k_high_order_next_cached<E, kWidth, kCachedP, false, decltype(mode)::value>), grid,
                             block, 0, launch_stream, eparams, mm, nw.U.ptr, d_bounds.ptr, d_pij.ptr, d_lij.ptr,
                             d_lij_next.ptr, d_V.ptr, last_s0, a.slice_flags);
        };
        launch_mode(std::integral_constant<int, kHoLight>{});
        hipLaunchKernelGGL(k_pij_repair<E>, grid, block, 0, launch_stream, mm, last_s0, d_pij.ptr, a.slice_flags);
        launch_mode(std::integral_constant<int, kHoHeavy>{});
        record_step6(mm, 1, false);
        return;
      }
    }
    if constexpr (DIM <= 2) {
      const uint32_t n_launch = mm.slice_end - mm.slice_begin;
      if (plan.step6_shares_slices(n_launch)) {
        hipLaunchKernelGGL((k_high_order_next_cached<E, kWidth, kWidth, true>), dim3(n_launch), block, 0,
                           launch_stream, eparams, mm, nw.U.ptr, d_bounds.ptr, d_pij.ptr, d_lij.ptr, d_lij_next.ptr,
                           V, last_s0, SliceFlags{unlimited, nullptr, nullptr});
        record_step6(mm, 1, true);
        return;
      }
    }
    if (plan.step6 == Step6::cached) {
      SliceFlags flags6 = a.tile_flags;
      flags6.unlimited = unlimited;
      hipLaunchKernelGGL((k_high_order_next_cached<E, kWidth, kCachedP>), grid, block, 0, launch_stream, eparams, mm,
                         nw.U.ptr, d_bounds.ptr, d_pij.ptr, d_lij.ptr, d_lij_next.ptr, V, last_s0, flags6);
    } else
      with_bool(plan.wide, [&](auto wide) {
        hipLaunchKernelGGL((k_high_order<E, false, decltype(wide)::value>), grid, block, 0, launch_stream, eparams,
                           mm, nw.U.ptr, d_bounds.ptr, d_pij.ptr, d_lij.ptr, d_lij_next.ptr,
                           FusedSadd{0., 0., nullptr});
      });
    record_step6(mm, 1, false);
  });
  if (plan.checked)
    sweep([&](const DeviceMesh &mm, dim3 grid) {
      hipLaunchKernelGGL(k_check_admissible<E>, grid, block, 0, launch_stream, eparams, mm, d_scalars.ptr,
                         (const double *)nw.U.ptr);
      hipLaunchKernelGGL(k_check_limiter<E>, grid, block, 0, launch_stream, eparams, mm, d_scalars.ptr,
                         (const double *)nw.U.ptr, (const double *)d_bounds.ptr, (const double *)d_pij.ptr,
                         (const double *)d_lij.ptr);
    });
  exchange_matrix(d_lij_next.ptr, true);
}

template <typename E>
void ryujin_hip_ctx::step7_high_order_last(const StepPlan &plan, const StepArgs<E::DIMENSION> &a)
{
  constexpr int DIM = E::DIMENSION;
  constexpr int kWidth = q1_stencil_width(DIM);
  constexpr int kLastChunk = DIM == 3 ? RYUJIN_LAST_CHUNK_3D : (DIM == 2 ? RYUJIN_LAST_CHUNK_2D : kWidth);
  const auto &eparams = eq_params<E>();
  const dim3 block(kBlock);
  const State &nw = a.nw;
  sweep([&](const DeviceMesh &mm, dim3 grid) {
    if (plan.step7 == StepPlan::Step7::last_cached)
      hipLaunchKernelGGL((k_high_order_last_cached<E, kWidth, kLastChunk>), grid, block, 0, launch_stream, eparams,
                         mm, nw.U.ptr, d_pij.ptr, d_lij.ptr, a.fused_sadd, a.fused_prec,
                         plan.step6_flags ? d_slice_unlimited.ptr : nullptr);
    else
      hipLaunchKernelGGL((k_high_order<E, true>), grid, block, 0, launch_stream, eparams, mm, nw.U.ptr,
                         d_bounds.ptr, d_pij.ptr, d_lij.ptr, d_lij_next.ptr, a.fused_sadd);
  });
  if (plan.checked)
    sweep([&](const DeviceMesh &mm, dim3 grid) {
      hipLaunchKernelGGL(k_check_admissible<E>, grid, block, 0, launch_stream, eparams, mm, d_scalars.ptr,
                         (const double *)nw.U.ptr);
    });
}

int ryujin_hip_ctx::finish_step(double *tau_out)
{
  HIP_CHECK(hipMemcpyAsync(h_scalars, d_scalars.ptr, sizeof(DeviceScalars), hipMemcpyDeviceToHost,
                           stream));
  HIP_CHECK(hipStreamSynchronize(stream));
  update_limited_fraction();

  if (timers_enabled) {
    for (int k = 0; k < 7; ++k) {
      float ms = 0.f;
      HIP_CHECK(hipEventElapsedTime(&ms, ev[k], ev[k + 1]));
      sweep_ms[k + 1] = ms;
    }
    sweep_ms[0] = 0.;
    if (last_plan.step2_split) {
      float ms = 0.f;
      HIP_CHECK(hipEventElapsedTime(&ms, ev[0], ev[8]));
      sweep_ms[0] = ms;
    }
    for (int k = 0; k < 8; ++k)
      sweep_ms_accum[k] += sweep_ms[k];
    ++sweep_updates_accum;
  }

  if (h_scalars->tau_invalid)
    return RYUJIN_ERR_TAU;
  *tau_out = h_scalars->tau;

  if (h_scalars->restart_needed) {
    if (params.id_violation_strategy == RYUJIN_IDV_WARN) {
      n_warnings++;
      return RYUJIN_WARN;
    }
    n_restarts++;
    return RYUJIN_RESTART;
  }
  return RYUJIN_OK;
}

template <typename E>
int ryujin_hip_ctx::step(int h_old, int stages, const int *h_stage, const double *w, int h_new,
                         double tau_in, double tau_max_in, double *tau_out)
{
  constexpr int DIM = E::DIMENSION;
  State &old = state(h_old);
  State &nw = state(h_new);
  if (h_old == h_new)
    throw HipError(RYUJIN_ERR_ARG, "old and new state vector must differ");
  nw.precomputed = false;

  const StepPlan plan = plan_step(plan_input<E>(stages));
  if (plan.unsupported)
    throw HipError(RYUJIN_ERR_UNSUPPORTED, plan.unsupported);
  if (plan.violated)
    throw HipError(RYUJIN_ERR_ARG, std::string("internal: ") + plan.violated);
  last_plan = plan;
  last_launches = LaunchLog{};
  pending_precompute = false;

  const bool use_device_tau = deferred && rk_stage > 0;
  struct ClearBegin {
    StepBegin &b;
    ~ClearBegin() { b = StepBegin{}; }
  } clear_begin{pending_begin};
  pending_begin = StepBegin{d_scalars.ptr,
                            tau_max_in,
                            tau_in,
                            (!deferred || rk_stage == 0) ? 1 : 0,
                            (deferred && rk_stage > 0) ? rk_stage - 1 : -1,
                            use_device_tau ? 1 : 0,
                            deferred ? rk_stage : 0};
  mark(0);
// ... 552 lines not shown
    host += first * K;
    std::vector<double> tmp(K == KP ? 0 : n * KP, 0.);
    if constexpr (kUpload) {
      for (size_t i = 0; i < n && K != KP; ++i)
        std::memcpy(&tmp[i * KP], &host[i * K], sizeof(double) * K);
      HIP_CHECK(hipMemcpy(dev, K == KP ? host : tmp.data(), n * KP * sizeof(double), hipMemcpyHostToDevice));
    } else {
      HIP_CHECK(hipMemcpy(K == KP ? host : tmp.data(), dev, n * KP * sizeof(double), hipMemcpyDeviceToHost));
      for (size_t i = 0; i < n && K != KP; ++i)
        std::memcpy(&host[i * K], &tmp[i * KP], sizeof(double) * K);
    }
  }
}

extern "C" {

const char *ryujin_hip_last_error(void)
{
  return g_error.c_str();
}

const char *ryujin_hip_version(void)
{
  return "ryujin_hip 0.4 (gfx950; Euler, Euler AEOS, shallow water, scalar conservation; SELL-64)";
}

void ryujin_hip_default_params(ryujin_hip_params *p, int equation, int dim)
{
  std::memset(p, 0, sizeof(*p));
  p->equation = equation;
  p->dim = dim;
  p->gamma = 7. / 5.;
  p->reference_density = 1.;
  p->vacuum_state_relaxation_small = 1.e2;
  p->vacuum_state_relaxation_large = 1.e4;
  p->gravity = 9.81;
  p->manning_friction_coefficient = 0.;
  p->reference_water_depth = 1.;
  p->dry_state_relaxation_factor = 2.e-1;
  p->dry_state_relaxation_small = 1.e2;
  p->dry_state_relaxation_large = 1.e4;
  p->cfl = 0.2;
  p->id_violation_strategy = RYUJIN_IDV_WARN;
  p->indicator_evc_factor = 1.;
  p->limiter_iterations = 2;
  p->limiter_newton_tolerance = 1.e-10;
  p->limiter_newton_max_iterations = 2;
  p->limiter_relaxation_factor = 1.;
  p->limiter_limit_on_kinetic_energy = 0;
  p->limiter_limit_on_square_velocity = 1;
  p->riemann_newton_max_iterations = 0;
  p->riemann_newton_tolerance = 1.e-10;
  p->eos = RYUJIN_EOS_POLYTROPIC_GAS;
  p->compute_strict_bounds = 1;
  p->eos_covolume_b = 0.;
  p->eos_q = 0.;
  p->eos_pinf = 0.;
  p->eos_vdw_a = 0.;
  p->eos_gas_constant_R = 287.052874;
  p->jwl_A = 6.3207e13;
  p->jwl_B = -4.472e9;
  p->jwl_R1 = 11.3;
  p->jwl_R2 = 1.13;
  p->jwl_omega = 0.8938;
  p->jwl_rho_0 = 1895.;
  p->jwl_q_0 = 0.;
  p->jwl_cv = 2487. / 1895.;
  p->sc_flux = RYUJIN_FLUX_BURGERS;
  p->sc_flux_polynomial[0][2] = 0.5;
  p->sc_derivative_approximation_delta = 1.e-10;
  p->sc_use_greedy_wavespeed = 0;
  p->sc_use_averaged_entropy = 0;
  p->sc_random_entropies = 0;
  p->system_scope_events = 0;
  p->debug_join_exchanges = 0;
  p->debug_bc_fold_max_slices = 0;
  p->debug_no_small_mesh_split = 0;
  p->debug_pij_storage = 0;
  p->debug_expensive_bounds_check = 0;
  p->debug_tile_map = 0;
  p->debug_band_stride = 0;
  p->debug_xcd_chunk = 0;
  p->debug_stencil_classes = 0;
  if (const char *e = std::getenv("RYUJIN_XCD_CHUNK"))
    p->debug_xcd_chunk = std::atoi(e);
  if (const char *e = std::getenv("RYUJIN_BAND_STRIDE"))
    p->debug_band_stride = std::atoi(e);
}

int ryujin_hip_comm_unique_id(char id[RYUJIN_HIP_UNIQUE_ID_BYTES])
{
  return guarded([&]() {
    static_assert(sizeof(ncclUniqueId) <= RYUJIN_HIP_UNIQUE_ID_BYTES, "unique id size");
    ncclUniqueId uid;
    NCCL_CHECK(ncclGetUniqueId(&uid));
    std::memset(id, 0, RYUJIN_HIP_UNIQUE_ID_BYTES);
    std::memcpy(id, &uid, sizeof(uid));
    return RYUJIN_OK;
  });
}

int ryujin_hip_comm_init(ryujin_hip_comm **comm, const char id[RYUJIN_HIP_UNIQUE_ID_BYTES], int rank,
                         int n_ranks, int device)
{
  return guarded([&]() {
    auto c = std::make_unique<ryujin_hip_comm>();
    c->rank = rank;
    c->n_ranks = n_ranks;
    c->device = device;
    HIP_CHECK(hipSetDevice(device));
    ncclUniqueId uid;
    std::memcpy(&uid, id, sizeof(uid));
    NCCL_CHECK(ncclCommInitRank(&c->comm, n_ranks, uid, rank));
    *comm = c.release();
    return RYUJIN_OK;
  });
}

int ryujin_hip_comm_init_local(ryujin_hip_comm **comms, int n_ranks, int device)
{
  return guarded([&]() {
    if (n_ranks < 1)
      throw HipError(RYUJIN_ERR_ARG, "n_ranks must be positive");
    auto *group = new LocalGroup(n_ranks, device);
    group->refs = n_ranks;
    for (int r = 0; r < n_ranks; ++r) {
      auto *c = new ryujin_hip_comm;
      c->rank = r;
      c->n_ranks = n_ranks;
      c->device = device;
      c->local = group;
      comms[r] = c;
    }
    return RYUJIN_OK;
  });
}

int ryujin_hip_comm_init_loopback(ryujin_hip_comm **comm, int rank, int n_ranks, int device)
{
  return guarded([&]() {
    if (!comm || n_ranks < 2 || rank < 0 || rank >= n_ranks)
      throw HipError(RYUJIN_ERR_ARG, "loopback communicator: 0 <= rank < n_ranks, n_ranks >= 2");
    auto *group = new LocalGroup(n_ranks, device);
    group->refs = 1;
    group->loopback = true;
    auto *c = new ryujin_hip_comm;
    c->rank = rank;
    c->n_ranks = n_ranks;
    c->device = device;
    c->local = group;
    *comm = c;
    return RYUJIN_OK;
  });
}

void ryujin_hip_comm_destroy(ryujin_hip_comm *comm)
{
  if (!comm)
    return;
  if (comm->local) {
    bool last;
    {
      std::lock_guard<std::mutex> lock(comm->local->mtx);
      last = --comm->local->refs == 0;
    }
    if (last)
// ... 379 lines not shown

int ryujin_hip_get_counters(ryujin_hip_ctx *ctx, unsigned *n_restarts, unsigned *n_warnings)
{
  *n_restarts = ctx->n_restarts;
  *n_warnings = ctx->n_warnings;
  return RYUJIN_OK;
}

int ryujin_hip_limiter_statistics(ryujin_hip_ctx *ctx, double *limited_slice_fraction, int *pij_stored,
                                  double *stored_slice_fraction)
{
  return guarded([&]() {
    if (!ctx)
      throw HipError(RYUJIN_ERR_ARG, "null context");
    if (limited_slice_fraction)
      *limited_slice_fraction = ctx->limited_fraction;
    if (pij_stored)
      *pij_stored = ctx->last_plan.pij_stored;
    if (stored_slice_fraction)
      *stored_slice_fraction = ctx->stored_fraction;
    return RYUJIN_OK;
  });
}

int ryujin_hip_tile_statistics(ryujin_hip_ctx *ctx, double *stored_fraction, double *read_fraction,
                               double *formed_by_step6_fraction)
{
  return guarded([&]() {
    if (!ctx)
      throw HipError(RYUJIN_ERR_ARG, "null context");
    const bool tiles = ctx->last_plan.per_tile();
    if (stored_fraction)
      *stored_fraction = tiles ? ctx->stored_fraction : 1.;
    if (read_fraction)
      *read_fraction = tiles ? ctx->tiles_needed_fraction : 1.;
    if (formed_by_step6_fraction)
      *formed_by_step6_fraction = tiles ? ctx->tiles_formed_fraction : 0.;
    return RYUJIN_OK;
  });
}

int ryujin_hip_layout_info(ryujin_hip_ctx *ctx, unsigned long long *n_tiles, unsigned long long *n_regular_tiles)
{
  return guarded([&]() {
    if (!ctx)
      throw HipError(RYUJIN_ERR_ARG, "null context");
    if (n_tiles)
      *n_tiles = ctx->L.slice_off[ctx->L.n_slices];
    if (n_regular_tiles)
      *n_regular_tiles = (ctx->d_tiles.n != 0 && tile_map_pays(ctx->dim)) ? ctx->L.n_regular_tiles : 0ull;
    return RYUJIN_OK;
  });
}

int ryujin_hip_chain_info(ryujin_hip_ctx *ctx, unsigned long long *n_chained_tiles,
                          unsigned long long *n_chained_entries)
{
  return guarded([&]() {
    if (!ctx)
      throw HipError(RYUJIN_ERR_ARG, "null context");
    const bool masks = ctx->dim == 3;
    if (n_chained_tiles)
      *n_chained_tiles = ctx->d_tiles.n == 0 ? 0ull : (masks ? ctx->L.n_chained_tiles : ctx->L.n_end_lane_tiles);
    if (n_chained_entries)
      *n_chained_entries = ctx->d_tiles.n == 0 ? 0ull : (masks ? ctx->L.n_chained_entries : 63ull * ctx->L.n_end_lane_tiles);
    return RYUJIN_OK;
  });
}

int ryujin_hip_stencil_class_info(ryujin_hip_ctx *ctx, unsigned long long *n_uniform_slices,
                                  unsigned long long *n_classes, double *uniform_entry_fraction)
{
  return guarded([&]() {
    if (!ctx)
      throw HipError(RYUJIN_ERR_ARG, "null context");
    const bool table = ctx->d_slice_class.n != 0;
    const uint64_t n_tiles = ctx->L.slice_off[ctx->L.n_slices];
    if (n_uniform_slices)
      *n_uniform_slices = table ? ctx->L.n_uniform_slices : 0ull;
    if (n_classes)
      *n_classes = table ? ctx->L.n_stencil_classes() : 0ull;
    if (uniform_entry_fraction)
      *uniform_entry_fraction = table && n_tiles != 0 ? (double)ctx->L.n_uniform_tiles / (double)n_tiles : 0.;
    return RYUJIN_OK;
  });
}

int ryujin_hip_debug_plan(ryujin_hip_ctx *ctx, int *out, int n)
{
  return guarded([&]() {
    if (!ctx || (n > 0 && !out) || n < 0)
      throw HipError(RYUJIN_ERR_ARG, "null context or output");
    const StepPlan &p = ctx->last_plan;
    const auto &log = ctx->last_launches;
    int v[RYUJIN_DEBUG_PLAN_LENGTH] = {(int)p.step2,
                                       p.step2_split,
                                       p.fast_riemann,
                                       p.diag_width,
                                       p.step4_single_walk,
                                       p.step4_has_stages,
                                       p.step4_friction,
                                       p.step4_stores_p,
                                       p.dg,
                                       (int)p.step5,
                                       (int)p.step5_groups,
                                       p.wide,
                                       p.has_V,
                                       p.pij_stored,
                                       p.tiles_predicted_from_history,
                                       (int)p.step6,
                                       p.step6_flags,
                                       (int)p.step7,
                                       p.fuse_precompute,
                                       p.checked,
                                       log.n_step5,
                                       log.n_step6};
    static_assert(22 + 5 * ryujin_hip_ctx::LaunchLog::kParts == RYUJIN_DEBUG_PLAN_LENGTH, "layout of the record");
    for (int q = 0; q < ryujin_hip_ctx::LaunchLog::kParts; ++q) {
      v[22 + 2 * q] = (int)log.step5[q].n_slices;
      v[23 + 2 * q] = (int)log.step5[q].grid_y;
      v[26 + 3 * q] = (int)log.step6[q].n_slices;
      v[27 + 3 * q] = (int)log.step6[q].grid_y;
      v[28 + 3 * q] = log.step6[q].shares_slices;
    }
    for (int q = 0; q < std::min(n, (int)RYUJIN_DEBUG_PLAN_LENGTH); ++q)
      out[q] = v[q];
    return (int)RYUJIN_DEBUG_PLAN_LENGTH;
  });
}

int ryujin_hip_debug_fetch(ryujin_hip_ctx *ctx, int what, double *out, size_t n_doubles)
{
  return guarded_ctx(ctx, [&]() {
    const auto &L = ctx->L;
    ctx->finish();
    auto fetch_matrix = [&](const double *dev, uint32_t n_comp) {
      if (n_doubles < L.nnz_owned_logical * n_comp)
        throw HipError(RYUJIN_ERR_ARG, "output buffer too small");
      std::vector<double> tmp(L.nnz_total * n_comp);
      HIP_CHECK(hipMemcpy(tmp.data(), dev, tmp.size() * sizeof(double), hipMemcpyDeviceToHost));
      L.gather_logical(tmp, n_comp, out);
    };
    switch (what) {
    case 0: fetch_matrix(ctx->d_dij.ptr, 1); break;
    case 1: fetch_matrix(ctx->d_lij.ptr, 1); break;
    case 2:
      ctx->ensure_pij();
      if (ctx->last_plan.pij_stored != 1)
        dispatch_equation(ctx->params.equation, ctx->dim, [&](auto tag) {
          using E = typename decltype(tag)::type;
          if constexpr (std::is_same<typename E::Params, EulerParams>::value ||
                        std::is_same<typename E::Params, EulerAeosParams>::value)
            ctx->template store_pij_for_debug<E>();
          return 0;
        });
      fetch_matrix(ctx->d_pij.ptr, (uint32_t)ctx->K);
      break;
    case 5: fetch_matrix(ctx->d_lij_next.ptr, 1); break;
    case 6:
    case 7:
    case 8: {
      const double *dev = what == 6 ? ctx->d_dij.ptr : (what == 7 ? ctx->d_lij.ptr : ctx->d_lij_next.ptr);
      const uint64_t n_ghost_entries = L.nnz_total - L.nnz_sell;
      if (n_doubles < L.nnz_owned_logical + n_ghost_entries)
        throw HipError(RYUJIN_ERR_ARG, "output buffer too small");
      std::vector<double> tmp(L.nnz_total);
      HIP_CHECK(hipMemcpy(tmp.data(), dev, tmp.size() * sizeof(double), hipMemcpyDeviceToHost));
      L.gather_logical(tmp, 1, out);
      std::copy(tmp.begin() + L.nnz_sell, tmp.end(), out + L.nnz_owned_logical);
      break;
    }
    case 9: {
      if (n_doubles < (size_t)L.n_relevant * ctx->K)
        throw HipError(RYUJIN_ERR_ARG, "output buffer too small");
      std::vector<double> tmp((size_t)L.n_relevant * ctx->KP);
      HIP_CHECK(hipMemcpy(tmp.data(), ctx->d_r.ptr, tmp.size() * sizeof(double), hipMemcpyDeviceToHost));
      for (uint32_t i = 0; i < L.n_relevant; ++i)
        for (int q = 0; q < ctx->K; ++q)
          out[(size_t)i * ctx->K + q] = tmp[(size_t)i * ctx->KP + q];
      break;
    }
    case 3: {
      if (n_doubles < (size_t)L.n_owned * ctx->NB)
        throw HipError(RYUJIN_ERR_ARG, "output buffer too small");
      std::vector<double> tmp((size_t)ctx->NB * ctx->mesh.bounds_stride);
      HIP_CHECK(hipMemcpy(tmp.data(), ctx->d_bounds.ptr, tmp.size() * sizeof(double),
                          hipMemcpyDeviceToHost));
      for (uint32_t i = 0; i < L.n_owned; ++i)
        for (int b = 0; b < ctx->NB; ++b)
          out[(size_t)i * ctx->NB + b] = tmp[(size_t)b * ctx->mesh.bounds_stride + i];
      break;
    }
    case 4: {
      if (n_doubles < (size_t)L.n_owned * ctx->K)
        throw HipError(RYUJIN_ERR_ARG, "output buffer too small");
      std::vector<double> tmp((size_t)L.n_relevant * ctx->KP);
      HIP_CHECK(hipMemcpy(tmp.data(), ctx->d_r.ptr, tmp.size() * sizeof(double),
                          hipMemcpyDeviceToHost));
      for (uint32_t i = 0; i < L.n_owned; ++i)
        for (int q = 0; q < ctx->K; ++q)
          out[(size_t)i * ctx->K + q] = tmp[(size_t)i * ctx->KP + q];
      break;
    }
    default: throw HipError(RYUJIN_ERR_ARG, "unknown debug_fetch selector");
    }
    return RYUJIN_OK;
  });
}

int ryujin_hip_debug_addresses(ryujin_hip_ctx *ctx, uint64_t out[8])
{
  return guarded([&]() {
    if (!ctx || !out)
      throw HipError(RYUJIN_ERR_ARG, "null argument");
    ctx->ensure_pij();
    const void *p[8] = {ctx->d_cols.ptr, ctx->d_cij.ptr, ctx->d_mij.ptr, ctx->d_dij.ptr,
                        ctx->d_lij.ptr,  ctx->d_lij_next.ptr, ctx->d_pij.ptr, ctx->d_idx_t.ptr};
    for (int q = 0; q < 8; ++q)
      out[q] = (uint64_t)(uintptr_t)p[q];
    return RYUJIN_OK;
  });
}

int ryujin_hip_debug_layout(const ryujin_hip_offline *offline, uint64_t *ptr, uint32_t *col,
                            uint64_t *transposed, const double *data, uint32_t n_comp, double *out)
{
  return guarded([&]() {
    SellLayout L;
    L.build(*offline);
    const RefView ref(*offline);
    std::vector<uint64_t> lptr((size_t)L.n_relevant + 1, 0);
    for (uint32_t i = 0; i < L.n_relevant; ++i)
      lptr[i + 1] = lptr[i] + ref.row_length(i);
    std::vector<uint64_t> logical_of(L.nnz_total, ~uint64_t(0));
    for (uint32_t i = 0; i < L.n_relevant; ++i)
      for (uint32_t c = 0; c < ref.row_length(i); ++c)
        logical_of[L.pos(i, c)] = lptr[i] + c;
    std::vector<double> dev;
    if (data && out)
      dev = L.scatter(*offline, data, n_comp);
    for (uint32_t i = 0; i < L.n_relevant; ++i)
      for (uint32_t c = 0; c < ref.row_length(i); ++c) {
        const uint64_t p = L.pos(i, c), e = lptr[i] + c;
        if (col)
          col[e] = L.cols[p];
        if (transposed)
          transposed[e] = logical_of[L.idx_t[p]];
        if (data && out)
          for (uint32_t d = 0; d < n_comp; ++d)
            out[e * n_comp + d] = dev[L.comp_pos(p, n_comp, d)];
      }
    if (ptr)
      std::copy(lptr.begin(), lptr.end(), ptr);
    return RYUJIN_OK;
  });
}

int ryujin_hip_debug_pow(int device, const double *x, const double *y, double *out, size_t n)
{
  return guarded([&]() {
    HIP_CHECK(hipSetDevice(device));
    DeviceBuffer<double> dx, dy, dout;
    dx.upload(x, n);
    dy.upload(y, n);
    dout.alloc(n);
    hipLaunchKernelGGL(k_debug_pow, dim3(grid_for(n)), dim3(kBlock), 0, nullptr, n, dx.ptr, dy.ptr,
                       dout.ptr);
    HIP_CHECK(hipGetLastError());
    HIP_CHECK(hipMemcpy(out, dout.ptr, n * sizeof(double), hipMemcpyDeviceToHost));
    return RYUJIN_OK;
  });
}

namespace
{
  __global__ void __launch_bounds__(kBlock)
  k_debug_function(const EulerParams PE, const ShallowWaterParams PS, const EulerAeosParams PA, const int which,
                   const size_t n, const double *__restrict__ in, double *__restrict__ out)
  {
    const size_t q = (size_t)blockIdx.x * blockDim.x + threadIdx.x;
    if (q >= n)
      return;
    if (which == RYUJIN_DEBUG_AEOS_RIEMANN) {
      using A = EulerAeos<1>;
      const double *v = in + q * 10;
      const A::RiemannData rd_i = A::make_riemann_data(PA, v[0], v[1], v[2], v[3], v[4]),
                           rd_j = A::make_riemann_data(PA, v[5], v[6], v[7], v[8], v[9]);
      const double r_i[A::RS] = {rd_i.rho, rd_i.p, rd_i.gamma, rd_i.a, rd_i.alpha, rd_i.alpha_hat, rd_i.u, 0.},
// ... 1374 lines not shown
```

### ryujin_amd/csrc/step_plan.hpp

```cpp
#ifndef RYUJIN_HIP_STEP_PLAN_HPP
#define RYUJIN_HIP_STEP_PLAN_HPP

#include <algorithm>
#include <cstdint>

namespace ryujin_hip
{
  enum class PlanEquation { euler, euler_aeos, scalar, shallow_water };

  constexpr uint32_t kPlanWavesPerBlock = 4;

  constexpr int q1_stencil_width(const int dim) { return dim == 1 ? 3 : (dim == 2 ? 9 : 27); }

  struct StepPlanInput {
    PlanEquation equation = PlanEquation::euler;
    int dim = 1;
    bool fusable_precompute = false;
    int stages = 0, limiter_iterations = 2;
    bool dg = false;
    uint32_t max_row_len = 0, n_slices = 0;
    int debug_pij_storage = 0;
    bool checked = false;
    double limited_fraction = 1.;
    double per_slice_max_limited = 1.;
    uint32_t resident_waves_step5 = 0, resident_waves_step6 = 0, bc_fold_max_slices = 0;
    bool pending_precompute = false;
    int riemann_newton_max_iterations = 0, rarefaction_power = 0;
    bool friction = false;
  };

  struct StepPlan {
    int dim = 1;
    uint32_t resident_waves_step5 = 0, resident_waves_step6 = 0;
    enum class Step2 {
      alpha_then_dij,
      dij_alpha_sc,
      records,
      dij_alpha
    } step2 = Step2::dij_alpha;
    bool step2_split = false;
    bool fast_riemann = false;
    int diag_width = 0;
    bool step4_single_walk = false, step4_has_stages = false, step4_friction = false, step4_stores_p = true;
    bool dg = false;
    enum class Step5 { none, stage0_per_tile, stage0_per_slice, stage0_groups, recompute, pij_lij } step5 = Step5::none;
    uint32_t step5_groups = 1;
    bool wide = false;
    bool has_V = false;
    int pij_stored = 1;
    bool tiles_predicted_from_history = false;
    enum class Step6 { none, per_slice, cached, high_order } step6 = Step6::none;
    bool step6_flags = false;
    enum class Step7 { none, last_cached, high_order } step7 = Step7::none;
    bool fuse_precompute = false;
    bool checked = false;
    const char *unsupported = nullptr, *violated = nullptr;

    bool per_slice() const { return pij_stored == 2; }
    bool per_tile() const { return pij_stored == 3; }

    uint32_t recompute_groups(const uint32_t grid_x) const
    {
      return std::min(4u, std::max(1u, resident_waves_step5 / std::max(1u, grid_x * kPlanWavesPerBlock)));
    }
    bool step6_shares_slices(const uint32_t n_launch_slices) const
    {
      return step6 == Step6::cached && dim <= 2 && !per_tile() &&
             n_launch_slices * kPlanWavesPerBlock <= resident_waves_step6;
    }
  };

  inline StepPlan plan_step(const StepPlanInput &in)
  {
    const bool is_euler = in.equation == PlanEquation::euler, is_aeos = in.equation == PlanEquation::euler_aeos;
    const bool is_scalar = in.equation == PlanEquation::scalar, is_sw = in.equation == PlanEquation::shallow_water;
    const int n_iterations = in.limiter_iterations;
    const uint32_t q1_width = (uint32_t)q1_stencil_width(in.dim);
    StepPlan p;
    p.dim = in.dim;
    p.resident_waves_step5 = in.resident_waves_step5;
    p.resident_waves_step6 = in.resident_waves_step6;
    p.checked = in.checked;
    p.dg = in.dg;
    p.wide = in.max_row_len > 64;

    p.fast_riemann = is_euler && in.riemann_newton_max_iterations == 0 && in.rarefaction_power > 0;
    if (is_aeos) {
      if (in.max_row_len > 32)
        p.unsupported = "euler aeos: stencils of more than 32 entries";
      p.step2 = StepPlan::Step2::alpha_then_dij;
    } else if (is_scalar)
      p.step2 = StepPlan::Step2::dij_alpha_sc;
    else if ((p.fast_riemann || is_sw) && in.max_row_len <= 32)
      p.step2 = StepPlan::Step2::records;
    else if (is_euler && in.max_row_len <= 32)
      p.step2 = StepPlan::Step2::alpha_then_dij;
    else
      p.step2 = StepPlan::Step2::dij_alpha;
    p.step2_split = p.step2 == StepPlan::Step2::alpha_then_dij || p.step2 == StepPlan::Step2::dij_alpha_sc;

    p.diag_width = in.max_row_len <= 3 ? 3 : (in.max_row_len <= 9 ? 9 : (in.max_row_len <= 27 ? 27 : 0));

    const bool recompute_p =
        is_euler && in.dim <= 2 && in.stages == 0 && n_iterations != 0 && !in.dg && in.max_row_len <= 64;
    const bool stage0_pij =
        (is_euler || is_aeos) && in.stages == 0 && n_iterations != 0 && !in.dg && in.max_row_len <= q1_width;

    p.step4_single_walk = is_sw && !in.dg && in.max_row_len <= (uint32_t)(in.dim == 1 ? 3 : 9);
    p.step4_has_stages = in.stages != 0;
    p.step4_friction = is_sw && in.friction;
    p.step4_stores_p = !(recompute_p || stage0_pij);

    const uint32_t step5_groups = std::min<uint32_t>(
        4u, in.resident_waves_step5 /
                std::max<uint32_t>(1u, (in.n_slices + kPlanWavesPerBlock - 1) / kPlanWavesPerBlock * kPlanWavesPerBlock));
    const int storage = in.debug_pij_storage;
    const bool selective = stage0_pij && n_iterations == 2 && step5_groups < 2 && storage >= 0 && !in.checked;
    const bool tile_store = in.dim <= 2 && selective && storage != 1;
    const bool per_slice =
        selective && !tile_store && (storage != 0 || in.limited_fraction <= in.per_slice_max_limited);
    p.pij_stored = per_slice ? 2 : (tile_store ? 3 : 1);
    p.tiles_predicted_from_history = tile_store && storage == 0;

    const bool two_passes = n_iterations == 2;
    if (n_iterations == 0)
      p.step5 = StepPlan::Step5::none;
    else if (stage0_pij) {
      p.step5 = tile_store ? StepPlan::Step5::stage0_per_tile
                           : (per_slice ? StepPlan::Step5::stage0_per_slice : StepPlan::Step5::stage0_groups);
      p.step5_groups = (tile_store || per_slice) ? 1u : std::max(1u, step5_groups);
      p.has_V = two_passes && p.step5_groups == 1;
    } else if (recompute_p)
      p.step5 = StepPlan::Step5::recompute;
    else {
      p.step5 = StepPlan::Step5::pij_lij;
      p.has_V = two_passes;
    }

    const bool cached = in.max_row_len <= q1_width;
    if (two_passes) {
      p.step6 = per_slice ? StepPlan::Step6::per_slice : (cached ? StepPlan::Step6::cached : StepPlan::Step6::high_order);
      p.step6_flags = per_slice || (cached && p.has_V);
    }
    if (n_iterations != 0)
      p.step7 = cached ? StepPlan::Step7::last_cached : StepPlan::Step7::high_order;

    p.fuse_precompute = in.fusable_precompute && in.pending_precompute && n_iterations != 0 &&
                        in.n_slices > in.bc_fold_max_slices && cached;

    if (p.per_tile() && !(p.has_V && p.step5 == StepPlan::Step5::stage0_per_tile && p.step5_groups == 1 && in.dim <= 2))
      p.violated = "step plan: P_ij per tile needs V_i, one wave per slice and dim <= 2";
    else if (p.per_slice() && !(p.has_V && p.step5 == StepPlan::Step5::stage0_per_slice))
      p.violated = "step plan: P_ij per slice needs V_i";
    else if (p.wide && p.step5 != StepPlan::Step5::none && p.step5 != StepPlan::Step5::pij_lij)
      p.violated = "step plan: rows of more than 64 entries need k_pij_lij<WIDE> in step 5";
    else if (p.checked && p.pij_stored != 1)
      p.violated = "step plan: the checked kernels read all of P_ij";
    return p;
  }
}

#endif
```

### ryujin_amd/module.py

```python
from __future__ import annotations

import ctypes as C

import numpy as np

from . import capi


class Restart(Exception):
    """Mirror of ryujin::Restart (source/hyperbolic_module.h:49-57)."""


class TauError(RuntimeError):
    """tau_max is NaN/inf/<=0 (AssertThrow at hyperbolic_module.template.h:573-576)."""


class StateVector:

    def __init__(self, module: "HyperbolicModule"):
        self.module = module
        h = C.c_int(-1)
        module._check(module._f("state_alloc")(module._ctx, C.byref(h)))
        self.handle = h.value

# ... 468 lines not shown
        n = C.c_size_t(0)
        fn = self._f("quantities_time_series")
        self._check(fn(self._ctx, manifold, None, 0, C.byref(n), 0))
        rows = np.zeros((n.value, 1 + 2 * self.k), dtype=np.float64)
        self._check(fn(self._ctx, manifold, capi.as_ptr(rows, capi.c_double_p), n.value, C.byref(n), int(bool(clear))))
        return rows

    def sadd(self, dst: StateVector, s: float, b: float, src: StateVector):
        self._check(self._f("sadd")(self._ctx, dst.handle, float(s), float(b), src.handle))

    @property
    def cfl(self) -> float:
        v = C.c_double()
        self._check(self._f("get_cfl")(self._ctx, C.byref(v)))
        return v.value

    @cfl.setter
    def cfl(self, value: float):
        self._check(self._f("set_cfl")(self._ctx, float(value)))

    @property
    def id_violation_strategy(self):
        return self._idv if hasattr(self, "_idv") else self.params.id_violation_strategy

    @id_violation_strategy.setter
    def id_violation_strategy(self, s: int):
        self._idv = s
        self._check(self._f("set_id_violation_strategy")(self._ctx, int(s)))

    def alpha(self) -> np.ndarray:
        a = np.empty(self.n_relevant, dtype=np.float64)
        self._check(self._f("get_alpha")(self._ctx, capi.as_ptr(a, capi.c_double_p)))
        return a

    def _counters(self):
        r, w = C.c_uint(), C.c_uint()
        self._check(self._f("get_counters")(self._ctx, C.byref(r), C.byref(w)))
        return r.value, w.value

    def n_restarts(self) -> int:
        return self._counters()[0]

    def n_warnings(self) -> int:
        return self._counters()[1]

    def exchange_info(self) -> dict:
        n_nbr, nx, nr = C.c_int(0), C.c_ulonglong(0), C.c_ulonglong(0)
        nbr = (C.c_int * 64)()
        self._check(self._f("exchange_info")(self._ctx, C.byref(n_nbr), nbr, 64, C.byref(nx), C.byref(nr)))
        return dict(neighbours=[nbr[q] for q in range(min(n_nbr.value, 64))], n_exchanges=nx.value,
                    n_allreduces=nr.value)

    def limiter_statistics(self) -> dict:
        f, stored, fs = C.c_double(1.0), C.c_int(1), C.c_double(1.0)
        fn = self._f("limiter_statistics")
        fn.argtypes = [C.c_void_p, C.POINTER(C.c_double), C.POINTER(C.c_int), C.POINTER(C.c_double)]
        self._check(fn(self._ctx, C.byref(f), C.byref(stored), C.byref(fs)))
        out = dict(limited_slice_fraction=f.value,
                   pij_stored={1: "everywhere", 2: "per slice", 3: "per tile"}.get(stored.value),
                   pij_stored_slice_fraction=fs.value)
        if stored.value == 3:
            a, b, c = C.c_double(1.0), C.c_double(1.0), C.c_double(0.0)
            self._check(self._lib.ryujin_hip_tile_statistics(self._ctx, C.byref(a), C.byref(b), C.byref(c)))
            out.update(tiles_stored_fraction=a.value, tiles_read_fraction=b.value, tiles_formed_by_step6_fraction=c.value)
        return out

    def layout_info(self) -> dict:
        n, r = C.c_ulonglong(0), C.c_ulonglong(0)
        self._check(self._lib.ryujin_hip_layout_info(self._ctx, C.byref(n), C.byref(r)))
        ch, ce = C.c_ulonglong(0), C.c_ulonglong(0)
        if hasattr(self._lib, "ryujin_hip_chain_info"):
            self._lib.ryujin_hip_chain_info.argtypes = [C.c_void_p, C.POINTER(C.c_ulonglong), C.POINTER(C.c_ulonglong)]
            self._check(self._lib.ryujin_hip_chain_info(self._ctx, C.byref(ch), C.byref(ce)))
        return dict(n_tiles=n.value, n_regular_tiles=r.value,
                    regular_tile_fraction=(r.value / n.value if n.value else 0.0),
                    n_chained_tiles=ch.value, chained_tile_fraction=(ch.value / n.value if n.value else 0.0),
                    chained_entry_fraction=(ce.value / (64.0 * n.value) if n.value else 0.0))

    def stencil_class_info(self) -> dict:
        n, k, f = C.c_ulonglong(0), C.c_ulonglong(0), C.c_double(0.0)
        self._check(self._lib.ryujin_hip_stencil_class_info(self._ctx, C.byref(n), C.byref(k), C.byref(f)))
        return dict(n_uniform_slices=n.value, n_classes=k.value, uniform_entry_fraction=f.value)

    PLAN_STEP2 = ("alpha_then_dij", "dij_alpha_sc", "records", "dij_alpha")
    PLAN_STEP5 = ("none", "stage0_per_tile", "stage0_per_slice", "stage0_groups", "recompute", "pij_lij")
    PLAN_STEP6 = ("none", "per_slice", "cached", "high_order")
    PLAN_STEP7 = ("none", "last_cached", "high_order")

    def last_plan(self) -> dict:
        n = 32
        v = (C.c_int * n)()
        rc = self._lib.ryujin_hip_debug_plan(self._ctx, v, n)
        if rc != n:
            self._check(rc if rc < 0 else capi.RYUJIN_ERR_ARG)
        flags = ("step2_split", "fast_riemann", None, "step4_single_walk", "step4_has_stages", "step4_friction",
                 "step4_stores_p", "dg", None, None, "wide", "has_V", None, "tiles_predicted_from_history", None,
                 "step6_flags", None, "fuse_precompute", "checked")
        out = dict(step2=self.PLAN_STEP2[v[0]], diag_width=v[3], step5=self.PLAN_STEP5[v[9]], step5_groups=v[10],
                   pij_stored=v[13], step6=self.PLAN_STEP6[v[15]], step7=self.PLAN_STEP7[v[17]])
        out.update({name: bool(v[1 + q]) for q, name in enumerate(flags) if name})
        out["step5_launches"] = [dict(n_slices=v[22 + 2 * q], grid_y=v[23 + 2 * q]) for q in range(min(v[20], 2))]
        out["step6_launches"] = [dict(n_slices=v[26 + 3 * q], grid_y=v[27 + 3 * q], shares_slices=bool(v[28 + 3 * q]))
                                 for q in range(min(v[21], 2))]
        return out

    def debug_fetch(self, what: str) -> np.ndarray:
        codes = {"dij": 0, "lij": 1, "pij": 2, "bounds": 3, "r": 4, "lij_next": 5,
                 "dij_all": 6, "lij_all": 7, "lij_next_all": 8, "r_all": 9}
        rs = self.offline.row_starts
        nnz_owned = int(rs[self.n_owned])
        nnz_all = int(rs[self.n_relevant])
        sizes = {"dij": nnz_owned, "lij": nnz_owned, "pij": nnz_owned * self.k,
                 "bounds": self.n_owned * self.n_bounds, "r": self.n_owned * self.k,
                 "lij_next": nnz_owned, "dij_all": nnz_all, "lij_all": nnz_all, "lij_next_all": nnz_all,
                 "r_all": self.n_relevant * self.k}
        out = np.empty(sizes[what], dtype=np.float64)
        self._check(self._f("debug_fetch")(self._ctx, codes[what], capi.as_ptr(out, capi.c_double_p),
                                           out.size))
        return out


class DeviceResidentTimeIntegrator:

    def __init__(self, module: "HyperbolicModule", scheme: str = "erk 33", cfl_min=0.45, cfl_max=0.90,
                 cfl_recovery_strategy: str = "bang bang control", dirichlet_fn=None, dirichlet=None):
        self.m, self.scheme = module, scheme
        self.cfl_min, self.cfl_max, self.cfl_recovery_strategy = cfl_min, cfl_max, cfl_recovery_strategy
        if dirichlet is not None and (dirichlet != "device" or dirichlet_fn is not None):
            raise ValueError("dirichlet is \"device\" or None, and excludes dirichlet_fn")
        self.dirichlet_fn, self.dirichlet = dirichlet_fn, dirichlet
        self.temp = [module.new_state_vector() for _ in range({"erk 43": 4, "erk 54": 5}.get(scheme, 3))]
        module.cfl = cfl_max

    def step(self, state: StateVector, t: float, t_final: float = np.finfo(np.float64).max):
        tau = self.m.time_step(self.scheme, state, self.temp, tau_max=t_final - t,
                               cfl_recovery=self.cfl_recovery_strategy, cfl_min=self.cfl_min, cfl_max=self.cfl_max,
                               t=t, dirichlet_fn=self.dirichlet_fn, dirichlet=self.dirichlet)
        return state, tau


class TimeIntegrator:

    def __init__(self, module: HyperbolicModule, scheme: str = "erk 33", cfl_min=0.45, cfl_max=0.90,
                 cfl_recovery_strategy: str = "bang bang control", dirichlet_fn=None):
        self.m = module
        self.scheme = scheme
        self.cfl_min, self.cfl_max = cfl_min, cfl_max
        self.cfl_recovery_strategy = cfl_recovery_strategy
        self.dirichlet_fn = dirichlet_fn
        n_temp = {"erk 43": 4, "erk 54": 5}.get(scheme, 3)
        self.temp = [module.new_state_vector() for _ in range(n_temp)]
        module.cfl = cfl_max

    def _prepare(self, sv, t):
        self.m.prepare_state_vector(sv, t, self.dirichlet_fn(t) if self.dirichlet_fn else None)

    def step(self, state: StateVector, t: float, t_final: float = np.finfo(np.float64).max):
        tau_max = t_final - t
        single = {"ssprk 22": self._ssprk22, "ssprk 33": self._ssprk33, "erk 11": self._erk11,
                  "erk 22": self._erk22, "erk 33": self._erk33, "erk 43": self._erk43,
                  "erk 54": self._erk54}[self.scheme]
        if self.cfl_recovery_strategy == "bang bang control":
            self.m.id_violation_strategy = capi.IDV_RAISE_EXCEPTION
            self.m.cfl = self.cfl_max
        try:
            return single(state, t, tau_max)
        except Restart:
            if self.cfl_recovery_strategy == "none":
                raise
            self.m.id_violation_strategy = capi.IDV_WARN
            self.m.cfl = self.cfl_min
            return single(state, t, tau_max)

    def _swap(self, state, idx):
        new = self.temp[idx]
        self.temp[idx] = state
        return new

    def _erk11(self, sv, t, tau_max):
        self._prepare(sv, t)
        tau = self.m.step(sv, [], [], self.temp[0], 0.0, tau_max)
        return self._swap(sv, 0), tau

    def _ssprk22(self, sv, t, tau_max):
        T = self.temp
        self._prepare(sv, t)
        tau = self.m.step(sv, [], [], T[0], 0.0, tau_max)
# ... 140 lines not shown
```

Baseline: 8890 MDoF-updates/s.

## Record per-slice limiter tile mask in step 6 to skip zero l_ij stores and reads

Step 6 now writes a per-slice bitmask of the off-diagonal tiles whose next limiter value is nonzero. It then elides the streaming stores of zeros into lij_next for owned, non-exported slices. Step 7 reads the mask and skips loading l_ij and the transposed tile descriptors for unnamed tiles, treating them as zero. This removes HBM traffic for the mostly-zero limiter matrix, at the cost of one extra word per slice and a stricter plan (2D, single-launch cached step 6). Debug fetch paths materialise the elided zeros.

```diff
diff --git a/include/ryujin_hip.h b/include/ryujin_hip.h
--- a/include/ryujin_hip.h
+++ b/include/ryujin_hip.h
@@ -103,6 +103,7 @@
   int debug_band_stride;
   int debug_xcd_chunk;
   int debug_stencil_classes;
+  int debug_next_tile_mask;
 } ryujin_hip_params;
 
 typedef struct ryujin_hip_offline {
@@ -218,10 +219,13 @@
                           unsigned long long *n_chained_entries);
 int ryujin_hip_stencil_class_info(ryujin_hip_ctx *ctx, unsigned long long *n_uniform_slices,
                                   unsigned long long *n_classes, double *uniform_entry_fraction);
+int ryujin_hip_next_tile_mask_info(ryujin_hip_ctx *ctx, int *active, unsigned long long *n_tiles,
+                                   unsigned long long *n_named);
 int ryujin_hip_tile_statistics(ryujin_hip_ctx *ctx, double *stored_fraction, double *read_fraction,
                                double *formed_by_step6_fraction);
 
 int ryujin_hip_debug_fetch(ryujin_hip_ctx *ctx, int what, double *out, size_t n_doubles);
+int ryujin_hip_debug_fill(ryujin_hip_ctx *ctx, int what, double value);
 #define RYUJIN_DEBUG_PLAN_LENGTH 32
 int ryujin_hip_debug_plan(ryujin_hip_ctx *ctx, int *out, int n);
 int ryujin_hip_set_timers(ryujin_hip_ctx *ctx, int enable);
diff --git a/ryujin_amd/capi.py b/ryujin_amd/capi.py
--- a/ryujin_amd/capi.py
+++ b/ryujin_amd/capi.py
@@ -66,6 +66,7 @@
         ("debug_pij_storage", C.c_int), ("debug_expensive_bounds_check", C.c_int),
         ("debug_tile_map", C.c_int), ("debug_band_stride", C.c_int),
         ("debug_xcd_chunk", C.c_int), ("debug_stencil_classes", C.c_int),
+        ("debug_next_tile_mask", C.c_int),
     ]
 
 
@@ -353,6 +354,7 @@
     "ryujin_hip_time_step_fn", "ryujin_hip_debug_addresses",
     "ryujin_hip_host_register", "ryujin_hip_host_unregister", "ryujin_hip_state_download_owned",
     "ryujin_hip_state_download_prepared", "ryujin_hip_layout_info", "ryujin_hip_chain_info", "ryujin_hip_stencil_class_info", "ryujin_hip_tile_statistics",
+    "ryujin_hip_next_tile_mask_info", "ryujin_hip_debug_fill",
     "ryujin_hip_default_params", "ryujin_hip_create", "ryujin_hip_destroy",
     "ryujin_hip_state_alloc", "ryujin_hip_state_free", "ryujin_hip_state_upload",
     "ryujin_hip_state_download", "ryujin_hip_state_download_precomputed", "ryujin_hip_state_integrals",
@@ -446,6 +448,11 @@
         if hasattr(lib, "ryujin_hip_stencil_class_info"):
             lib.ryujin_hip_stencil_class_info.argtypes = [vp, C.POINTER(C.c_ulonglong), C.POINTER(C.c_ulonglong),
                                                           C.POINTER(C.c_double)]
+        if hasattr(lib, "ryujin_hip_debug_fill"):
+            lib.ryujin_hip_debug_fill.argtypes = [vp, C.c_int, C.c_double]
+        if hasattr(lib, "ryujin_hip_next_tile_mask_info"):
+            lib.ryujin_hip_next_tile_mask_info.argtypes = [vp, c_int_p, C.POINTER(C.c_ulonglong),
+                                                           C.POINTER(C.c_ulonglong)]
         lib.ryujin_hip_tile_statistics.argtypes = [vp, C.POINTER(C.c_double), C.POINTER(C.c_double), C.POINTER(C.c_double)]
         lib.ryujin_hip_host_register.argtypes = [vp, C.c_void_p, C.c_size_t]
         lib.ryujin_hip_host_unregister.argtypes = [vp, C.c_void_p]
diff --git a/ryujin_amd/csrc/kernels_euler.hpp b/ryujin_amd/csrc/kernels_euler.hpp
--- a/ryujin_amd/csrc/kernels_euler.hpp
+++ b/ryujin_amd/csrc/kernels_euler.hpp
@@ -417,15 +417,17 @@
   RYUJIN_DEV void batch_fence() { __builtin_amdgcn_sched_barrier(0); }
 
   template <bool USE, int N>
-  RYUJIN_DEV void transposed_positions(const DeviceMesh &M, const RowCtx &r, const int c0, uint32_t (&tpos)[N])
-  {
+  RYUJIN_DEV void transposed_positions(const DeviceMesh &M, const RowCtx &r, const int c0, uint32_t (&tpos)[N],
+                                       const uint32_t cols = ~0u)
+  {
+    auto asked = [&](const int k) { return (uint32_t)(c0 + k) < r.width && ((cols >> ((c0 + k) & 31)) & 1u) != 0u; };
     if constexpr (USE) {
       if (M.tiles != nullptr) {
         int4 raw[N];
 #pragma unroll
         for (int k = 0; k < N; ++k) {
           raw[k] = int4{kTileIrregular, 0, 0, 0};
-          if ((uint32_t)(c0 + k) < r.width)
+          if (asked(k))
             raw[k] = load_tile_desc(M.tiles + ((uint64_t)r.base + c0 + k));
         }
         batch_fence();
@@ -433,7 +435,7 @@
 #pragma unroll
         for (int k = 0; k < N; ++k) {
           tpos[k] = 0;
-          if ((uint32_t)(c0 + k) < r.width) {
+          if (asked(k)) {
             const int32_t delta = __builtin_amdgcn_readfirstlane(raw[k].x);
             const uint32_t ta = (uint32_t)__builtin_amdgcn_readfirstlane(raw[k].y);
             const uint32_t tb = (uint32_t)__builtin_amdgcn_readfirstlane(raw[k].z);
@@ -444,7 +446,7 @@
         if (any_irregular) {
 #pragma unroll
           for (int k = 0; k < N; ++k)
-            if ((uint32_t)(c0 + k) < r.width && __builtin_amdgcn_readfirstlane(raw[k].x) == kTileIrregular)
+            if (asked(k) && __builtin_amdgcn_readfirstlane(raw[k].x) == kTileIrregular)
               tpos[k] = M.idx_t[((uint64_t)r.base + c0 + k) * 64 + r.lane];
         }
 #pragma unroll
@@ -456,7 +458,7 @@
 #pragma unroll
     for (int k = 0; k < N; ++k) {
       tpos[k] = 0;
-      if ((uint32_t)(c0 + k) < r.width)
+      if (asked(k))
         tpos[k] = M.idx_t[((uint64_t)r.base + c0 + k) * 64 + r.lane];
     }
 #pragma unroll
diff --git a/ryujin_amd/csrc/kernels_limiter.hpp b/ryujin_amd/csrc/kernels_limiter.hpp
--- a/ryujin_amd/csrc/kernels_limiter.hpp
+++ b/ryujin_amd/csrc/kernels_limiter.hpp
@@ -742,7 +742,15 @@
   struct SliceFlags {
     uint8_t *unlimited, *first_stored, *todo;
     uint32_t *needed_tiles;
+    uint32_t *next_tiles;
+    uint32_t next_tiles_elide;
   };
+
+  RYUJIN_DEV uint32_t slice_next_tiles(const uint32_t *next_tiles, const uint32_t slice)
+  {
+    typedef const uint32_t __attribute__((address_space(4))) *const_ptr;
+    return (uint32_t)__builtin_amdgcn_readfirstlane((int)*(const_ptr)(uintptr_t)(next_tiles + slice));
+  }
 
 #ifndef RYUJIN_GATHER_GROUP_3D
 #define RYUJIN_GATHER_GROUP_3D 6
@@ -783,7 +791,8 @@
   RYUJIN_DEV void last_cached_slice(const typename E::Params &P, const DeviceMesh &M, const RowCtx &r,
                                     double *__restrict__ new_U, const double *__restrict__ pij,
                                     const double *__restrict__ lij, const FusedSadd &F, const FusedPrecompute &FP,
-                                    const uint8_t *__restrict__ slice_unlimited = nullptr)
+                                    const uint8_t *__restrict__ slice_unlimited = nullptr,
+                                    const uint32_t *__restrict__ next_tiles = nullptr)
   {
     constexpr int K = E::K;
     const bool row_active = r.len > 1;
@@ -800,22 +809,27 @@
     double l[MAXW];
     uint32_t needed = 0;
     const bool known_unlimited = slice_unlimited != nullptr && slice_unlimited[r.slice] != 0;
+    uint32_t cols = ~0u;
+    if constexpr (MAXW <= 10) {
+      if (next_tiles != nullptr)
+        cols = slice_next_tiles(next_tiles, r.slice);
+    }
 #pragma unroll
     for (int c = 1; c < MAXW; ++c)
       l[c] = 0.;
-    if (!known_unlimited) {
+    if (!known_unlimited && cols != 0u) {
       constexpr int CH = MAXW - 1 < 9 ? MAXW - 1 : RYUJIN_GATHER_GROUP_3D;
 #pragma unroll
       for (int c0 = 1; c0 < MAXW; c0 += CH) {
         uint32_t tpos[CH];
-        transposed_positions<tile_map_pays<E::DIMENSION>(), CH>(M, r, c0, tpos);
+        transposed_positions<tile_map_pays<E::DIMENSION>(), CH>(M, r, c0, tpos, cols);
         batch_fence();
         double l_a[CH], l_b[CH];
 #pragma unroll
         for (int k = 0; k < CH; ++k) {
           const int c = c0 + k;
           l_a[k] = l_b[k] = 0.;
-          if (c < MAXW && (uint32_t)c < r.width) {
+          if (c < MAXW && (uint32_t)c < r.width && ((cols >> c) & 1u)) {
             l_a[k] = lij[(uint32_t)(((uint64_t)r.base + c) * 64 + r.lane)];
             l_b[k] = lij[tpos[k]];
           }
@@ -829,8 +843,11 @@
 #pragma unroll
         for (int k = 0; k < CH; ++k) {
           const int c = c0 + k;
-          if (c < MAXW && (uint32_t)c < r.width)
+          if (c < MAXW && (uint32_t)c < r.width && ((cols >> c) & 1u)) {
             l[c] = (row_active && (uint32_t)c < r.len) ? lmin(l_a[k], l_b[k]) : 0.;
+            if (next_tiles != nullptr)
+              l[c] = l_a[k] == 0. ? 0. : l[c];
+          }
         }
       }
 #pragma unroll
@@ -889,12 +906,13 @@
   __global__ void __launch_bounds__(kBlock, (MAXW > 9 ? RYUJIN_OCC_LAST_3D : 1))
   k_high_order_last_cached(const typename E::Params P, const DeviceMesh M, double *__restrict__ new_U,
                            const double *__restrict__ pij, const double *__restrict__ lij, const FusedSadd F,
-                           const FusedPrecompute FP, const uint8_t *__restrict__ slice_unlimited = nullptr)
+                           const FusedPrecompute FP, const uint8_t *__restrict__ slice_unlimited = nullptr,
+                           const uint32_t *__restrict__ next_tiles = nullptr)
   {
     const RowCtx r = row_context(M);
     if (!r.valid)
       return;
-    last_cached_slice<E, MAXW, CHUNK>(P, M, r, new_U, pij, lij, F, FP, slice_unlimited);
+    last_cached_slice<E, MAXW, CHUNK>(P, M, r, new_U, pij, lij, F, FP, slice_unlimited, next_tiles);
   }
 
   constexpr int kHoPlain = 0, kHoLight = 1, kHoHeavy = 2;
@@ -916,6 +934,10 @@
     constexpr int NB = E::NB;
     static_assert(!SPLIT || CP == MAXW, "the split variant caches the whole row");
     static_assert(!SPLIT || MODE == kHoPlain, "small meshes keep the stored P_ij");
+    constexpr bool kNextTiles = !SPLIT && MODE == kHoPlain && MAXW <= 10;
+    bool elide = false;
+    if constexpr (kNextTiles)
+      elide = W.next_tiles != nullptr && W.next_tiles_elide != 0u;
     const bool row_active = r.len > 1;
     const uint32_t i = row_active ? r.row : (r.row < M.n_owned ? r.row : M.n_owned - 1);
     const uint32_t *__restrict__ idx_t = M.idx_t;
@@ -1050,6 +1072,9 @@
       }
       if (W.unlimited != nullptr && r.lane == 0 && (!SPLIT || group == 0))
         W.unlimited[r.slice] = slice_limited ? 0 : 1;
+      if constexpr (kNextTiles)
+        if (W.next_tiles != nullptr && r.lane == 0)
+          W.next_tiles[r.slice] = needed;
       if constexpr (kTileMode)
         if (tiles && r.lane == 0 && (!SPLIT || group == 0))
           tiles_remember<MAXW>(W, r.slice, needed);
@@ -1058,10 +1083,12 @@
         if (row_active) {
           if (!SPLIT || group == 0)
             store_state<K>(new_U, i, U_i_new);
-#pragma unroll
-          for (int c = 1; c < MAXW; ++c)
-            if ((uint32_t)c < r.len && (!SPLIT || (uint32_t)(c - 1) % kWavesPerBlock == group))
-              st_stream(lij_next + ((r.base + c) * 64 + r.lane), 0.);
+          if (!elide) {
+#pragma unroll
+            for (int c = 1; c < MAXW; ++c)
+              if ((uint32_t)c < r.len && (!SPLIT || (uint32_t)(c - 1) % kWavesPerBlock == group))
+                st_stream(lij_next + ((r.base + c) * 64 + r.lane), 0.);
+          }
         }
         return;
       }
@@ -1160,6 +1187,9 @@
             needed |= 1u << c;
         }
       }
+      if constexpr (kNextTiles)
+        if (W.next_tiles != nullptr && r.lane == 0)
+          W.next_tiles[r.slice] = needed;
 #pragma unroll
       for (int c = 1; c < MAXW; ++c) {
         if (c < CP) {
@@ -1197,7 +1227,7 @@
         continue;
       const bool lane_on = row_active && (uint32_t)c < r.len;
       if (!((needed >> c) & 1u)) {
-        if (lane_on)
+        if (lane_on && !elide)
           st_stream(lij_next + ((r.base + c) * 64 + r.lane), 0.);
         continue;
       }
@@ -1241,6 +1271,19 @@
           const double old_l_ij = lmin(lij[pos], lij[idx_t[pos]]);
           st_stream(lij_next + (pos), (1. - old_l_ij) * new_l_ij);
         });
+  }
+
+  __global__ void __launch_bounds__(kBlock)
+  k_fill_unnamed_tiles(const DeviceMesh M, const uint32_t *__restrict__ next_tiles, double *__restrict__ lij)
+  {
+    const uint32_t slice = M.slice_begin + blockIdx.x * kWavesPerBlock + (threadIdx.x >> 6);
+    if (slice >= M.slice_end)
+      return;
+    const RowCtx r = row_context_of_slice(M, slice);
+    const uint32_t named = next_tiles[slice];
+    for (uint32_t c = 1; c < r.width && c < 32u; ++c)
+      if (!((named >> c) & 1u) && c < r.len)
+        lij[((uint64_t)r.base + c) * 64 + r.lane] = 0.;
   }
 
   template <typename E>
diff --git a/ryujin_amd/csrc/ryujin_hip.hip b/ryujin_amd/csrc/ryujin_hip.hip
--- a/ryujin_amd/csrc/ryujin_hip.hip
+++ b/ryujin_amd/csrc/ryujin_hip.hip
@@ -477,6 +477,7 @@
   }
   DeviceBuffer<uint8_t> d_slice_unlimited, d_slice_first_stored, d_slice_todo;
   DeviceBuffer<uint32_t> d_slice_needed;
+  DeviceBuffer<uint32_t> d_slice_next_tiles;
   double limited_fraction = 1., stored_fraction = 1.;
   unsigned int seen_sampled_slices = 0, seen_sampled_limited = 0, seen_sampled_stored = 0;
   unsigned int seen_sampled_tiles = 0, seen_sampled_tiles_stored = 0;
@@ -1278,7 +1279,9 @@
   in.dg = dg;
   in.max_row_len = L.max_row_len;
   in.n_slices = L.n_slices;
+  in.n_export_slices = exch.n_nbr != 0 ? n_export_slices : 0u;
   in.debug_pij_storage = params.debug_pij_storage;
+  in.debug_next_tile_mask = params.debug_next_tile_mask;
   in.checked = params.debug_expensive_bounds_check != 0;
   in.limited_fraction = limited_fraction;
   in.per_slice_max_limited = (double)RYUJIN_PER_SLICE_MAX_LIMITED;
@@ -1418,6 +1421,8 @@
     d_slice_needed.alloc(L.n_slices);
     HIP_CHECK(hipMemsetAsync(d_slice_needed.ptr, 0xff, (size_t)L.n_slices * sizeof(uint32_t), launch_stream));
   }
+  if (plan.next_tile_mask && d_slice_next_tiles.n == 0)
+    d_slice_next_tiles.alloc(L.n_slices);
 }
 
 template <typename E>
@@ -1594,6 +1599,9 @@
     if (plan.step6 == Step6::cached) {
       SliceFlags flags6 = a.tile_flags;
       flags6.unlimited = unlimited;
+      flags6.next_tiles = plan.next_tile_mask ? d_slice_next_tiles.ptr : nullptr;
+      flags6.next_tiles_elide =
+          plan.next_tiles_elided && (exch.n_nbr == 0 || mm.slice_begin >= n_export_slices) ? 1u : 0u;
       hipLaunchKernelGGL((k_high_order_next_cached<E, kWidth, kCachedP>), grid, block, 0, launch_stream, eparams, mm,
                          nw.U.ptr, d_bounds.ptr, d_pij.ptr, d_lij.ptr, d_lij_next.ptr, V, last_s0, flags6);
     } else
@@ -1628,7 +1636,8 @@
     if (plan.step7 == StepPlan::Step7::last_cached)
       hipLaunchKernelGGL((k_high_order_last_cached<E, kWidth, kLastChunk>), grid, block, 0, launch_stream, eparams,
                          mm, nw.U.ptr, d_pij.ptr, d_lij.ptr, a.fused_sadd, a.fused_prec,
-                         plan.step6_flags ? d_slice_unlimited.ptr : nullptr);
+                         plan.step6_flags ? d_slice_unlimited.ptr : nullptr,
+                         plan.next_tile_mask ? (const uint32_t *)d_slice_next_tiles.ptr : (const uint32_t *)nullptr);
     else
       hipLaunchKernelGGL((k_high_order<E, true>), grid, block, 0, launch_stream, eparams, mm, nw.U.ptr,
                          d_bounds.ptr, d_pij.ptr, d_lij.ptr, d_lij_next.ptr, a.fused_sadd);
@@ -2347,6 +2356,7 @@
   p->debug_band_stride = 0;
   p->debug_xcd_chunk = 0;
   p->debug_stencil_classes = 0;
+  p->debug_next_tile_mask = 0;
   if (const char *e = std::getenv("RYUJIN_XCD_CHUNK"))
     p->debug_xcd_chunk = std::atoi(e);
   if (const char *e = std::getenv("RYUJIN_BAND_STRIDE"))
@@ -2892,6 +2902,35 @@
       *n_classes = table ? ctx->L.n_stencil_classes() : 0ull;
     if (uniform_entry_fraction)
       *uniform_entry_fraction = table && n_tiles != 0 ? (double)ctx->L.n_uniform_tiles / (double)n_tiles : 0.;
+    return RYUJIN_OK;
+  });
+}
+
+int ryujin_hip_next_tile_mask_info(ryujin_hip_ctx *ctx, int *active, unsigned long long *n_tiles,
+                                   unsigned long long *n_named)
+{
+  return guarded_ctx(ctx, [&]() {
+    const auto &L = ctx->L;
+    const bool on = ctx->last_plan.next_tile_mask && ctx->d_slice_next_tiles.n == L.n_slices;
+    std::vector<uint32_t> words(on ? L.n_slices : 0u);
+    if (on) {
+      ctx->finish();
+      HIP_CHECK(hipMemcpy(words.data(), ctx->d_slice_next_tiles.ptr, words.size() * sizeof(uint32_t),
+                          hipMemcpyDeviceToHost));
+    }
+    unsigned long long tiles = 0, named = 0;
+    for (uint32_t s = 0; s < L.n_slices; ++s) {
+      const uint32_t width = L.slice_off[s + 1] - L.slice_off[s];
+      const uint32_t off_diagonal = width > 1 ? width - 1 : 0u;
+      tiles += off_diagonal;
+      named += on ? (unsigned long long)__builtin_popcount(words[s] & ~1u) : off_diagonal;
+    }
+    if (active)
+      *active = on ? 1 : 0;
+    if (n_tiles)
+      *n_tiles = tiles;
+    if (n_named)
+      *n_named = named;
     return RYUJIN_OK;
   });
 }
@@ -2944,6 +2983,17 @@
   return guarded_ctx(ctx, [&]() {
     const auto &L = ctx->L;
     ctx->finish();
+    auto materialise_zeros = [&](double *dev) {
+      if (!ctx->last_plan.next_tiles_elided || ctx->last_plan.step6 == StepPlan::Step6::none)
+        return;
+      DeviceMesh mm = ctx->mesh;
+      mm.slice_begin = 0;
+      mm.slice_end = L.n_slices;
+      hipLaunchKernelGGL(k_fill_unnamed_tiles, dim3((L.n_slices + kWavesPerBlock - 1) / kWavesPerBlock), dim3(kBlock), 0,
+                         ctx->stream, mm, (const uint32_t *)ctx->d_slice_next_tiles.ptr, dev);
+      HIP_CHECK(hipGetLastError());
+      HIP_CHECK(hipStreamSynchronize(ctx->stream));
+    };
     auto fetch_matrix = [&](const double *dev, uint32_t n_comp) {
       if (n_doubles < L.nnz_owned_logical * n_comp)
         throw HipError(RYUJIN_ERR_ARG, "output buffer too small");
@@ -2953,7 +3003,10 @@
     };
     switch (what) {
     case 0: fetch_matrix(ctx->d_dij.ptr, 1); break;
-    case 1: fetch_matrix(ctx->d_lij.ptr, 1); break;
+    case 1:
+      materialise_zeros(ctx->d_lij.ptr);
+      fetch_matrix(ctx->d_lij.ptr, 1);
+      break;
     case 2:
       ctx->ensure_pij();
       if (ctx->last_plan.pij_stored != 1)
@@ -2970,6 +3023,8 @@
     case 6:
     case 7:
     case 8: {
+      if (what == 7)
+        materialise_zeros(ctx->d_lij.ptr);
       const double *dev = what == 6 ? ctx->d_dij.ptr : (what == 7 ? ctx->d_lij.ptr : ctx->d_lij_next.ptr);
       const uint64_t n_ghost_entries = L.nnz_total - L.nnz_sell;
       if (n_doubles < L.nnz_owned_logical + n_ghost_entries)
@@ -3014,6 +3069,22 @@
     }
     default: throw HipError(RYUJIN_ERR_ARG, "unknown debug_fetch selector");
     }
+    return RYUJIN_OK;
+  });
+}
+
+int ryujin_hip_debug_fill(ryujin_hip_ctx *ctx, int what, double value)
+{
+  return guarded_ctx(ctx, [&]() {
+    if (what != 5)
+      throw HipError(RYUJIN_ERR_ARG, "unknown debug_fill selector");
+    ctx->finish();
+    const auto &L = ctx->L;
+    std::vector<double> tmp(L.nnz_total);
+    HIP_CHECK(hipMemcpy(tmp.data(), ctx->d_lij_next.ptr, tmp.size() * sizeof(double), hipMemcpyDeviceToHost));
+    for (uint32_t s = 0; s < L.n_slices; ++s)
+      std::fill(tmp.begin() + ((size_t)L.slice_off[s] + 1) * 64, tmp.begin() + (size_t)L.slice_off[s + 1] * 64, value);
+    HIP_CHECK(hipMemcpy(ctx->d_lij_next.ptr, tmp.data(), tmp.size() * sizeof(double), hipMemcpyHostToDevice));
     return RYUJIN_OK;
   });
 }
diff --git a/ryujin_amd/csrc/step_plan.hpp b/ryujin_amd/csrc/step_plan.hpp
--- a/ryujin_amd/csrc/step_plan.hpp
+++ b/ryujin_amd/csrc/step_plan.hpp
@@ -19,7 +19,9 @@
     int stages = 0, limiter_iterations = 2;
     bool dg = false;
     uint32_t max_row_len = 0, n_slices = 0;
+    uint32_t n_export_slices = 0;
     int debug_pij_storage = 0;
+    int debug_next_tile_mask = 0;
     bool checked = false;
     double limited_fraction = 1.;
     double per_slice_max_limited = 1.;
@@ -52,6 +54,8 @@
     enum class Step6 { none, per_slice, cached, high_order } step6 = Step6::none;
     bool step6_flags = false;
     enum class Step7 { none, last_cached, high_order } step7 = Step7::none;
+    bool next_tile_mask = false;
+    bool next_tiles_elided = false;
     bool fuse_precompute = false;
     bool checked = false;
     const char *unsupported = nullptr, *violated = nullptr;
@@ -69,6 +73,28 @@
              n_launch_slices * kPlanWavesPerBlock <= resident_waves_step6;
     }
   };
+
+  inline bool some_launch_shares_slices(const StepPlan &p, const uint32_t n_slices, const uint32_t n_export_slices)
+  {
+    const uint32_t n_export = std::min(n_export_slices, n_slices);
+    return (n_export != 0 && p.step6_shares_slices(n_export)) ||
+           (n_slices > n_export && p.step6_shares_slices(n_slices - n_export));
+  }
+
+  inline const char *next_tile_mask_violated(const StepPlan &p, const uint32_t n_slices, const uint32_t n_export_slices)
+  {
+    if (!p.next_tile_mask)
+      return p.next_tiles_elided ? "step plan: zeros are elided under the tile mask only" : nullptr;
+    if (p.step6 != StepPlan::Step6::cached || p.dim > 2)
+      return "step plan: the tile mask needs the single-launch cached step 6, dim <= 2";
+    if (some_launch_shares_slices(p, n_slices, n_export_slices))
+      return "step plan: the tile mask needs one wave per slice in every launch of step 6";
+    if (p.step7 != StepPlan::Step7::last_cached)
+      return "step plan: the tile mask needs the cached step 7";
+    if (p.checked)
+      return "step plan: the checked kernels read all of l_ij";
+    return nullptr;
+  }
 
   inline StepPlan plan_step(const StepPlanInput &in)
   {
@@ -145,6 +171,11 @@
     if (n_iterations != 0)
       p.step7 = cached ? StepPlan::Step7::last_cached : StepPlan::Step7::high_order;
 
+    p.next_tile_mask = in.debug_next_tile_mask >= 0 && p.step6 == StepPlan::Step6::cached && in.dim <= 2 &&
+                       !some_launch_shares_slices(p, in.n_slices, in.n_export_slices) &&
+                       p.step7 == StepPlan::Step7::last_cached && !in.checked;
+    p.next_tiles_elided = p.next_tile_mask && in.debug_next_tile_mask == 0;
+
     p.fuse_precompute = in.fusable_precompute && in.pending_precompute && n_iterations != 0 &&
                         in.n_slices > in.bc_fold_max_slices && cached;
 
@@ -156,6 +187,8 @@
       p.violated = "step plan: rows of more than 64 entries need k_pij_lij<WIDE> in step 5";
     else if (p.checked && p.pij_stored != 1)
       p.violated = "step plan: the checked kernels read all of P_ij";
+    else if (const char *v = next_tile_mask_violated(p, in.n_slices, in.n_export_slices))
+      p.violated = v;
     return p;
   }
 }
diff --git a/ryujin_amd/module.py b/ryujin_amd/module.py
--- a/ryujin_amd/module.py
+++ b/ryujin_amd/module.py
@@ -574,6 +574,11 @@
         self._check(self._lib.ryujin_hip_stencil_class_info(self._ctx, C.byref(n), C.byref(k), C.byref(f)))
         return dict(n_uniform_slices=n.value, n_classes=k.value, uniform_entry_fraction=f.value)
 
+    def next_tile_mask_info(self) -> dict:
+        a, n, k = C.c_int(0), C.c_ulonglong(0), C.c_ulonglong(0)
+        self._check(self._lib.ryujin_hip_next_tile_mask_info(self._ctx, C.byref(a), C.byref(n), C.byref(k)))
+        return dict(active=bool(a.value), n_tiles=n.value, n_named=k.value)
+
     PLAN_STEP2 = ("alpha_then_dij", "dij_alpha_sc", "records", "dij_alpha")
     PLAN_STEP5 = ("none", "stage0_per_tile", "stage0_per_slice", "stage0_groups", "recompute", "pij_lij")
     PLAN_STEP6 = ("none", "per_slice", "cached", "high_order")
@@ -595,6 +600,9 @@
         out["step6_launches"] = [dict(n_slices=v[26 + 3 * q], grid_y=v[27 + 3 * q], shares_slices=bool(v[28 + 3 * q]))
                                  for q in range(min(v[21], 2))]
         return out
+
+    def debug_fill(self, what: str, value: float) -> None:
+        self._check(self._lib.ryujin_hip_debug_fill(self._ctx, {"lij_next": 5}[what], float(value)))
 
     def debug_fetch(self, what: str) -> np.ndarray:
         codes = {"dij": 0, "lij": 1, "pij": 2, "bounds": 3, "r": 4, "lij_next": 5,
```

Result: faster. 9097 MDoF-updates/s, median of 6 (+2.3%).
